# Godotcoffee/AlignGraph2

Hardware: AMD Instinct MI355X
Metric: aligned-read-bases/sec through PAGraph build+traverse (higher is better)
Workload: dtype u32

## Files before the change

aligngraph2_amd/csrc/hip/k2_sort.hip:

```cpp
#include <stdlib.h>

#include "pag_device.hpp"

namespace pagdev {

#ifndef SORT_ST
#define SORT_ST 1024
#endif
#ifndef SORT_ROUNDS
#define SORT_ROUNDS 5
#endif
constexpr int ST = SORT_ST;
constexpr int SW = ST / 64;
constexpr int SROUNDS = SORT_ROUNDS;
constexpr int STILE = ST * SROUNDS;
constexpr int SMAXR = 256;

constexpr int HT = 256;
constexpr int HW = HT / 64;
constexpr int HV = STILE / (4 * HT);
static_assert(STILE % (4 * HT) == 0, "a tile is a whole number of 16-byte loads per thread");

__global__ __launch_bounds__(HT) void sort_hist(const uint32_t *__restrict__ keys, uint64_t n, int shift, uint32_t rmask,
                                                uint32_t *__restrict__ hist, uint32_t n_tiles, int aligned) {
    __shared__ uint32_t h[2][HW][SMAXR];
    const uint32_t w = threadIdx.x >> 6;
    uint4 nx[HV];
    auto request = [&](uint32_t tile) {
        const uint64_t base = (uint64_t)tile * STILE;
        if (aligned && tile < n_tiles && base + STILE <= n) {
            const uint4 *src = (const uint4 *)(keys + base);
#pragma unroll
            for (int r = 0; r < HV; ++r) nx[r] = src[r * HT + threadIdx.x];
        }
    };
    for (uint32_t i = threadIdx.x; i < 2 * HW * SMAXR; i += HT) (&h[0][0][0])[i] = 0;
    request(blockIdx.x);
    __syncthreads();
    uint32_t buf = 0;
    for (uint32_t tile = blockIdx.x; tile < n_tiles; tile += gridDim.x, buf ^= 1u) {
        const uint64_t base = (uint64_t)tile * STILE;
        uint32_t *hw = h[buf][w];
        if (aligned && base + STILE <= n) {
            uint4 cur[HV];
#pragma unroll
            for (int r = 0; r < HV; ++r) cur[r] = nx[r];
            request(tile + gridDim.x);
#pragma unroll
            for (int r = 0; r < HV; ++r) {
                atomicAdd(&hw[(cur[r].x >> shift) & rmask], 1u);
                atomicAdd(&hw[(cur[r].y >> shift) & rmask], 1u);
                atomicAdd(&hw[(cur[r].z >> shift) & rmask], 1u);
                atomicAdd(&hw[(cur[r].w >> shift) & rmask], 1u);
            }
        } else {
            request(tile + gridDim.x);
            for (uint32_t j = threadIdx.x; j < (uint32_t)STILE; j += HT)
                if (base + j < n) atomicAdd(&hw[(keys[base + j] >> shift) & rmask], 1u);
        }
        __syncthreads();
        for (uint32_t d = threadIdx.x; d <= rmask; d += HT) {
            uint32_t c = 0;
#pragma unroll
            for (int ww = 0; ww < HW; ++ww) {
                c += h[buf][ww][d];
                h[buf][ww][d] = 0;
            }
            hist[(uint64_t)d * n_tiles + tile] = c;
        }
    }
}

struct ScatterStage {
    uint64_t goff[SMAXR];
    uint32_t skey[STILE];
#ifdef SORT_TWO_PLANE
    uint32_t sval_lo[STILE], sval_hi[STILE];
#else
    uint64_t sval[STILE];
#endif
};
struct ScatterLds {
    uint32_t wcnt[SW][SMAXR + 1];
    uint32_t dstart[SMAXR];
    ScatterStage stage[2];
};
static_assert(SW == 16 || SW == 8, "the wave prefix below scans groups of SW lanes inside a DPP row");
static_assert(sizeof(ScatterLds) <= 160 * 1024, "LDS");
static_assert(STILE >= SW * SMAXR, "match words alias the payload staging buffer");

__device__ __forceinline__ uint32_t group_incl_sum(uint32_t v, uint32_t pos) {
    uint32_t t;
    t = (uint32_t)__builtin_amdgcn_update_dpp(0, (int)v, 0x111, 0xF, 0xF, true);
    v += (SW == 16 || pos >= 1u) ? t : 0u;
    t = (uint32_t)__builtin_amdgcn_update_dpp(0, (int)v, 0x112, 0xF, 0xF, true);
    v += (SW == 16 || pos >= 2u) ? t : 0u;
    t = (uint32_t)__builtin_amdgcn_update_dpp(0, (int)v, 0x114, 0xF, 0xF, true);
    v += (SW == 16 || pos >= 4u) ? t : 0u;
    if (SW == 16) v += (uint32_t)__builtin_amdgcn_update_dpp(0, (int)v, 0x118, 0xF, 0xF, true);
    return v;
}

__device__ __forceinline__ uint64_t scatter_tile(uint32_t block, uint32_t n_blocks, uint32_t it) {
    if (n_blocks % 8u != 0u) return (uint64_t)it * n_blocks + block;
    const uint32_t per_xcd = n_blocks / 8u, x = block & 7u, slot = block >> 3;
    return ((uint64_t)it * 8u + x) * per_xcd + slot;
}

#ifdef SORT_WAVES_PER_EU
#define SORT_BOUNDS __launch_bounds__(ST, SORT_WAVES_PER_EU)
#else
#define SORT_BOUNDS __launch_bounds__(ST)
#endif
template <int BITS>
__global__ SORT_BOUNDS void sort_scatter(const uint32_t *__restrict__ keys, const uint64_t *__restrict__ vals,
                                                  uint32_t *__restrict__ okeys, uint64_t *__restrict__ ovals, uint64_t n,
                                                  int shift, const uint64_t *__restrict__ hist_scan, uint32_t n_tiles) {
    __shared__ ScatterLds L;
    constexpr uint32_t rmask = (1u << BITS) - 1u;
    const uint32_t lane = lane_id(), w = threadIdx.x >> 6;
    const uint32_t n_iter = (n_tiles + gridDim.x - 1) / gridDim.x;

    uint32_t nkey[SROUNDS];
    uint64_t nval[SROUNDS];
    uint64_t ngbase = 0;
    auto request = [&](uint64_t tile) {
        const uint64_t wb = tile * STILE + (uint64_t)w * (64 * SROUNDS);
        if (threadIdx.x <= rmask && tile < n_tiles) ngbase = hist_scan[(uint64_t)threadIdx.x * n_tiles + tile];
#pragma unroll
        for (int r = 0; r < SROUNDS; ++r) {
            const uint64_t i = wb + (uint64_t)r * 64 + lane;
            const bool valid = tile < n_tiles && i < n;
            nkey[r] = valid ? keys[i] : 0u;
            nval[r] = valid ? vals[i] : 0ull;
        }
    };
    request(scatter_tile(blockIdx.x, gridDim.x, 0));

    const uint32_t last_count = (uint32_t)(n - (uint64_t)(n_tiles - 1u) * STILE);
    auto write_out = [&](const ScatterStage &B, uint32_t count) {
        if (count == (uint32_t)STILE) {
#pragma unroll
            for (int r = 0; r < SROUNDS; ++r) {
                const uint32_t p = (uint32_t)r * ST + threadIdx.x;
                const uint32_t kx = B.skey[p];
                const uint64_t dst = B.goff[(kx >> shift) & rmask] + p;
                okeys[dst] = kx;
#ifdef SORT_TWO_PLANE
                ovals[dst] = (uint64_t)B.sval_lo[p] | ((uint64_t)B.sval_hi[p] << 32);
#else
                ovals[dst] = B.sval[p];
#endif
            }
        } else {
            for (uint32_t p = threadIdx.x; p < count; p += ST) {
                const uint32_t kx = B.skey[p];
                const uint64_t dst = B.goff[(kx >> shift) & rmask] + p;
                okeys[dst] = kx;
#ifdef SORT_TWO_PLANE
                ovals[dst] = (uint64_t)B.sval_lo[p] | ((uint64_t)B.sval_hi[p] << 32);
#else
                ovals[dst] = B.sval[p];
#endif
            }
        }
    };

    bool pending = false;
    uint32_t pending_count = 0;
    uint32_t buf = 0;
    for (uint32_t it = 0; it < n_iter; ++it) {
        const uint64_t tile = scatter_tile(blockIdx.x, gridDim.x, it);
        uint32_t key[SROUNDS];
        uint64_t val[SROUNDS];
#pragma unroll
        for (int r = 0; r < SROUNDS; ++r) {
            key[r] = nkey[r];
            val[r] = nval[r];
        }
        const uint64_t gbase = ngbase;
        if (it + 1 < n_iter) request(scatter_tile(blockIdx.x, gridDim.x, it + 1));
        if (pending) write_out(L.stage[buf ^ 1u], pending_count);
        pending = false;
        if (tile >= n_tiles) continue;

        ScatterStage &B = L.stage[buf];
        const uint64_t tile_base = tile * STILE;
        const uint64_t wave_base = tile_base + (uint64_t)w * (64 * SROUNDS);
#ifdef SORT_TWO_PLANE
        unsigned long long *match = (unsigned long long *)&B.sval_lo[0] + (size_t)w * (rmask + 1u);
#else
        unsigned long long *match = (unsigned long long *)&B.sval[0] + (size_t)w * (rmask + 1u);
#endif
#pragma unroll
        for (int i = 0; i < SMAXR / 64; ++i) L.wcnt[w][i * 64 + lane] = 0;
#pragma unroll
        for (uint32_t i = lane; i <= rmask; i += 64) match[i] = 0ull;
        uint32_t rk[SROUNDS];
#pragma unroll
        for (int r = 0; r < SROUNDS; ++r) {
            const uint64_t i = wave_base + (uint64_t)r * 64 + lane;
            const bool valid = i < n;
            const uint32_t d = (key[r] >> shift) & rmask;
            if (valid) atomicOr(&match[d], 1ull << lane);
            const uint64_t peers = valid ? match[d] : 0ull;
            if (valid) match[d] = 0ull;
            const uint32_t before = __popcll(peers & lanemask_lt());
            const uint32_t base = valid ? L.wcnt[w][d] : 0u;
            if (valid && before == 0) L.wcnt[w][d] = base + (uint32_t)__popcll(peers);
            rk[r] = base + before;
        }

        __syncthreads();
        uint32_t *dtot = (uint32_t *)&B.goff[0];
#pragma unroll
        for (int j = 0; j < SMAXR * SW / ST; ++j) {
            const uint32_t d = (uint32_t)j * (ST / SW) + threadIdx.x / SW, ww = threadIdx.x % SW;
            const uint32_t c = L.wcnt[ww][d];
            const uint32_t incl = group_incl_sum(c, ww);
            L.wcnt[ww][d] = incl - c;
            if (ww == SW - 1u) dtot[d] = incl;
        }
        __syncthreads();
        if (w == 0) {
            const uint32_t t0 = dtot[4 * lane], t1 = dtot[4 * lane + 1], t2 = dtot[4 * lane + 2], t3 = dtot[4 * lane + 3];
            uint32_t tot;
            const uint32_t ex = wave_excl_sum(t0 + t1 + t2 + t3, &tot);
            L.dstart[4 * lane] = ex;
            L.dstart[4 * lane + 1] = ex + t0;
            L.dstart[4 * lane + 2] = ex + t0 + t1;
            L.dstart[4 * lane + 3] = ex + t0 + t1 + t2;
        }
        __syncthreads();
#ifdef SORT_LOOKBACK_PROBE
        if (threadIdx.x <= rmask) {
            uint32_t *rows = (uint32_t *)(hist_scan + (uint64_t)(rmask + 1u) * n_tiles);
            __hip_atomic_store(&rows[tile * (rmask + 1u) + threadIdx.x], dtot[threadIdx.x] | 0x40000000u, __ATOMIC_RELAXED, __HIP_MEMORY_SCOPE_AGENT);
            uint32_t acc = 0;
            for (uint32_t b = 1; b <= (uint32_t)SORT_LOOKBACK_PROBE; ++b) {
                const uint64_t t2 = tile >= b ? tile - b : 0;
                acc += __hip_atomic_load(&rows[t2 * (rmask + 1u) + threadIdx.x], __ATOMIC_RELAXED, __HIP_MEMORY_SCOPE_AGENT);
            }
            if (acc == 0xFFFFFFFFu) L.dstart[threadIdx.x] += 1u;
        }
        __syncthreads();
#endif
        if (threadIdx.x <= rmask) B.goff[threadIdx.x] = gbase - L.dstart[threadIdx.x];

#pragma unroll
        for (int r = 0; r < SROUNDS; ++r) {
            const uint64_t i = wave_base + (uint64_t)r * 64 + lane;
            if (i < n) {
                const uint32_t d = (key[r] >> shift) & rmask;
                const uint32_t p = L.dstart[d] + L.wcnt[w][d] + rk[r];
                B.skey[p] = key[r];
#ifdef SORT_TWO_PLANE
                B.sval_lo[p] = (uint32_t)val[r];
                B.sval_hi[p] = (uint32_t)(val[r] >> 32);
#else
                B.sval[p] = val[r];
#endif
            }
        }
        __syncthreads();
        pending = true;
        pending_count = tile == (uint64_t)n_tiles - 1u ? last_count : (uint32_t)STILE;
        buf ^= 1u;
    }
    if (pending) write_out(L.stage[buf ^ 1u], pending_count);
}

static int scatter_blocks_cus(int dev) {
    static int cus_of[64] = {0};
    int &c = cus_of[dev & 63];
    if (c == 0 && hipDeviceGetAttribute(&c, hipDeviceAttributeMultiprocessorCount, dev) != hipSuccess) c = 256;
    return c > 0 ? c : 256;
}

static size_t sort_align256(size_t x) { return (x + 255) & ~(size_t)255; }

size_t sort_tmp_bytes(uint64_t n) {
    uint64_t n_tiles = (n + STILE - 1) / STILE;
    if (n_tiles == 0) n_tiles = 1;
    uint64_t cells = (uint64_t)SMAXR * n_tiles;
#ifdef SORT_LOOKBACK_PROBE
    return sort_align256(cells * 4) + 2 * sort_align256(cells * 8) + sort_align256(scan_tmp_bytes(cells)) + 256;
#else
    return sort_align256(cells * 4) + sort_align256(cells * 8) + sort_align256(scan_tmp_bytes(cells)) + 256;
#endif
}

int sort_pairs(uint32_t *k0, uint64_t *v0, uint32_t *k1, uint64_t *v1, uint64_t n, int key_bits, void *tmp,
               int *result_in_0, hipStream_t s, float *ms_dominant_kernel, int *n_passes, int first_bit) {
    *result_in_0 = 1;
    if (ms_dominant_kernel) *ms_dominant_kernel = 0.f;
    if (n_passes) *n_passes = 0;
    if (n == 0 || key_bits <= 0) return PAG_OK;
    uint64_t n_tiles64 = (n + STILE - 1) / STILE;
    if (n_tiles64 > 0x7FFFFFFFull) {
        set_error("sort: too many tiles");
        return PAG_EINVAL;
    }
    uint32_t n_tiles = (uint32_t)n_tiles64;
    int passes = (key_bits + 7) / 8;
    int bits = (key_bits + passes - 1) / passes;
    char *p = (char *)tmp;
    uint32_t *hist = (uint32_t *)p;
    uint64_t cells = (uint64_t)SMAXR * n_tiles;
    p += sort_align256(cells * 4);
    uint64_t *hist_scan = (uint64_t *)p;
    p += sort_align256(cells * 8);
    void *scan_tmp = p;

    static int scatter_blocks_of[64] = {0};
    int dev = 0;
    PAG_HIP_TRY(hipGetDevice(&dev));
    int &scatter_blocks = scatter_blocks_of[dev & 63];
    if (scatter_blocks == 0) {
        int cus = 0, per_cu = 0;
        PAG_HIP_TRY(hipDeviceGetAttribute(&cus, hipDeviceAttributeMultiprocessorCount, dev));
        PAG_HIP_TRY(hipOccupancyMaxActiveBlocksPerMultiprocessor(&per_cu, sort_scatter<8>, ST, 0));
        scatter_blocks = cus * (per_cu > 0 ? per_cu : 1);
    }
    const uint32_t scatter_grid = n_tiles < (uint32_t)scatter_blocks ? n_tiles : (uint32_t)scatter_blocks;
    const int hist_per_cu = 8;
    const int hist_blocks = scatter_blocks_cus(dev) * hist_per_cu;
    const bool timed = ms_dominant_kernel != nullptr;
    static thread_local hipEvent_t ev_sets[64][2 * 8];
    static thread_local bool ev_ready[64] = {false};
    hipEvent_t *ev = ev_sets[dev & 63];
    if (timed && !ev_ready[dev & 63]) {
        for (int i = 0; i < 2 * 8; ++i) PAG_HIP_TRY(hipEventCreate(&ev[i]));
        ev_ready[dev & 63] = true;
    }
    uint32_t *ka = k0, *kb = k1;
    uint64_t *va = v0, *vb = v1;
    int in0 = 1;
    for (int pass = 0; pass < passes; ++pass) {
        int shift = first_bit + pass * bits;
        int b = key_bits - pass * bits < bits ? key_bits - pass * bits : bits;
        uint32_t rmask = (1u << b) - 1u;
        uint64_t used = (uint64_t)(rmask + 1) * n_tiles;
        const uint32_t hist_grid = n_tiles < (uint32_t)hist_blocks ? n_tiles : (uint32_t)hist_blocks;
        sort_hist<<<dim3(hist_grid), dim3(HT), 0, s>>>(ka, n, shift, rmask, hist, n_tiles, ((uintptr_t)ka & 15u) == 0 ? 1 : 0);
        int rc = scan_u32_to_u64(hist, hist_scan, used, nullptr, scan_tmp, s);
        if (rc != PAG_OK) return rc;
        if (timed) PAG_HIP_TRY(hipEventRecord(ev[2 * pass], s));
        switch (b) {
#define PAG_SCATTER(B)                                                                                              \
    case B:                                                                                                         \
        sort_scatter<B><<<dim3(scatter_grid), dim3(ST), 0, s>>>(ka, va, kb, vb, n, shift, hist_scan, n_tiles);      \
        break;
            PAG_SCATTER(1) PAG_SCATTER(2) PAG_SCATTER(3) PAG_SCATTER(4) PAG_SCATTER(5) PAG_SCATTER(6) PAG_SCATTER(7) PAG_SCATTER(8)
#undef PAG_SCATTER
        }
        if (timed) PAG_HIP_TRY(hipEventRecord(ev[2 * pass + 1], s));
        uint32_t *tk = ka;
        ka = kb;
        kb = tk;
        uint64_t *tv = va;
        va = vb;
        vb = tv;
        in0 = !in0;
    }
    PAG_HIP_TRY(hipGetLastError());
    if (timed) {
        PAG_HIP_TRY(hipStreamSynchronize(s));
        float tot = 0.f;
        for (int pass = 0; pass < passes; ++pass) {
            float ms = 0.f;
            PAG_HIP_TRY(hipEventElapsedTime(&ms, ev[2 * pass], ev[2 * pass + 1]));
            tot += ms;
        }
        *ms_dominant_kernel = tot / passes;
    }
    if (n_passes) *n_passes = passes;
    *result_in_0 = in0;
    return PAG_OK;
}

}
```

aligngraph2_amd/csrc/hip/k5_travel_host.hip:

```cpp
#include <algorithm>
#include <atomic>
#include <chrono>
#include <cmath>
#include <cstdio>
#include <cstdlib>
#include <cstring>
#include <deque>
#include <string>
#include <thread>
#include <unordered_set>
#include <vector>

#include "pag_graph_impl.hpp"
#include "walk_config.hpp"
#include "walk_stitch.hpp"
#include "walker_grid.hpp"

using namespace pagdev;

namespace {

#include "trav_prepare_host.hpp"
#include "walk_session_jobs.hpp"
#include "walk_session_rounds.hpp"
#include "walk_session_loop.hpp"


}


extern "C" {

uint64_t pag_debug_edit_distance(const char *a, const char *b) { return edit_distance(a, b); }
uint64_t pag_debug_mapper_d2s(const uint32_t *len, uint64_t n, int64_t idx, int64_t pos) { return Mapper(len, n).dualToSingle(idx, pos); }
void pag_debug_mapper_s2d(const uint32_t *len, uint64_t n, uint64_t single, int64_t *idx, int64_t *pos) {
    auto d = Mapper(len, n).singleToDual(single);
    *idx = d.first;
    *pos = d.second;
}
uint64_t pag_debug_mapper_extra(const uint32_t *len, uint64_t n) { return Mapper(len, n).starts.back(); }

const pag_path_node *pag_travel_path_oriented(const pag_graph *g, uint64_t ctg_index, int forward, uint64_t *len) {
    const uint64_t slot = 2 * ctg_index + (forward ? 0 : 1);
    if (!g || slot >= g->path_valid.size() || !g->path_valid[slot]) {
        if (len) *len = 0;
        return nullptr;
    }
    if (len) *len = g->path_len[slot];
    if (slot < g->path_ptr.size() && g->path_ptr[slot]) return g->path_ptr[slot];
    return g->path_store + g->path_off[slot];
}

const char *pag_travel_dump_text(const pag_graph *g, uint64_t ctg_index, int forward, uint64_t *bytes) {
    const uint64_t slot = 2 * ctg_index + (forward ? 0 : 1);
    if (bytes) *bytes = 0;
    if (!g || slot >= g->path_valid.size() || !g->path_valid[slot] || slot >= g->text_ptr.size() || !g->text_ptr[slot]) return nullptr;
    if (bytes) *bytes = g->text_len[slot];
    return g->text_ptr[slot];
}

const pag_path_node *pag_travel_path(const pag_graph *g, uint64_t ctg_index, uint64_t *len) {
    if (g && 2 * ctg_index + 1 < g->path_valid.size() && !g->path_valid[2 * ctg_index]) return pag_travel_path_oriented(g, ctg_index, 0, len);
    return pag_travel_path_oriented(g, ctg_index, 1, len);
}

int pag_debug_succ_sizes(const pag_graph *g, uint64_t *n_pos, uint64_t *n_succ) {
    if (!g || !g->tg_ready || !n_pos || !n_succ) return PAG_EINVAL;
    *n_pos = g->tg.n_pos;
    *n_succ = g->tg.n_succ;
    return PAG_OK;
}
int pag_debug_succ(const pag_graph *g, uint32_t *succ_off, void *recs) {
    if (!g || !g->tg_ready || !succ_off || !recs) return PAG_EINVAL;
    PAG_HIP_TRY(hipSetDevice(g->device));
    PAG_HIP_TRY(hipMemcpy(succ_off, g->tg.succ_off, (g->tg.n_pos + 1) * 4, hipMemcpyDeviceToHost));
    PAG_HIP_TRY(hipMemcpy(recs, g->tg.succ, g->tg.n_succ * sizeof(SuccRec), hipMemcpyDeviceToHost));
    return PAG_OK;
}

int pag_debug_trav_vertices(const pag_graph *g, uint32_t *code, uint64_t *pos) {
    if (!g || !g->tg_ready || !code || !pos) return PAG_EINVAL;
    PAG_HIP_TRY(hipSetDevice(g->device));
    const TravGraph &G = g->tg;
    std::vector<uint32_t> uold(G.n_pos), vnode(G.n_pos), ncode(G.n_nodes);
    PAG_HIP_TRY(hipMemcpy(uold.data(), G.uold, G.n_pos * 4, hipMemcpyDeviceToHost));
    PAG_HIP_TRY(hipMemcpy(vnode.data(), G.vnode, G.n_pos * 4, hipMemcpyDeviceToHost));
    PAG_HIP_TRY(hipMemcpy(ncode.data(), G.ncode, G.n_nodes * 4, hipMemcpyDeviceToHost));
    PAG_HIP_TRY(hipMemcpy(pos, G.upos, G.n_pos * 8, hipMemcpyDeviceToHost));
    for (uint64_t u = 0; u < G.n_pos; ++u) code[u] = ncode[vnode[uold[u]]];
    return PAG_OK;
}

int64_t pag_successors(const pag_graph *g, uint32_t code, uint64_t pos, pag_succ *out, uint64_t cap) {
    if (!g || !g->tg_ready || (!out && cap)) return PAG_EINVAL;
    PAG_HIP_TRY(hipSetDevice(g->device));
    if (g->view_pruned || g->regional) {
        set_error("pag_successors: the prepared view was cut for given traversals (pag_travel_prepare_for / a regional graph): its lists are restricted to what those traversals can examine");
        return PAG_ERANGE;
    }
    void *d = nullptr;
    const uint64_t room = std::min<uint64_t>(cap, g->tg.n_succ);
    PAG_HIP_TRY(hipMalloc(&d, 16 + room * sizeof(pag_succ)));
    unsigned long long *d_n = (unsigned long long *)d;
    void *d_recs = (char *)d + 16;
    int rc = trav_successors_of(g->tg, code, pos, d_recs, room, d_n, g->stream);
    unsigned long long n = 0;
    if (rc == PAG_OK && (hipMemcpyAsync(&n, d_n, 8, hipMemcpyDeviceToHost, g->stream) != hipSuccess || hipStreamSynchronize(g->stream) != hipSuccess)) rc = PAG_EFAULT;
    if (rc == PAG_OK && n == ~0ull) {
        set_error("pag_successors: the graph holds no vertex with that k-mer and position");
        rc = PAG_EINVAL;
    } else if (rc == PAG_OK && n == ~1ull) {
        set_error("pag_successors: that vertex's list is a marker record");
        rc = PAG_ERANGE;
    } else if (rc == PAG_OK && std::min<uint64_t>(n, room) &&
               hipMemcpy(out, d_recs, std::min<uint64_t>(n, room) * sizeof(pag_succ), hipMemcpyDeviceToHost) != hipSuccess) {
        rc = PAG_EFAULT;
    }
    hipFree(d);
    return rc == PAG_OK ? (int64_t)n : rc;
}

int pag_travel_prepare(pag_graph *g, const pag_seqs *ctgs, const uint32_t *ref_len, uint64_t n_refs, const pag_travel_params *prm, double *ms) {
    return pag_travel_prepare_for(g, ctgs, nullptr, ref_len, n_refs, prm, ms);
}
int pag_travel_prepare_for(pag_graph *g, const pag_seqs *ctgs, const int32_t *orient, const uint32_t *ref_len, uint64_t n_refs,
                           const pag_travel_params *prm, double *ms) {
    if (!g || !ctgs || !prm || (!ref_len && n_refs)) return PAG_EINVAL;
    PAG_HIP_TRY(hipSetDevice(g->device));
    TravGraph G{};
    return trav_prepare_graph(g, ctgs->len, ctgs->n_seqs, ref_len, n_refs, prm->deviation, prm->error_rate, &G, ms, orient, prm->start_split);
}
int pag_travel_view_sizes(const pag_graph *g, uint64_t *n_nodes, uint64_t *n_pos, uint64_t *n_edges, uint64_t *n_succ, int *cut, uint64_t *fallbacks) {
    if (!g || !g->tg_ready) return PAG_EINVAL;
    if (n_nodes) *n_nodes = g->view_counts[0];
    if (n_pos) *n_pos = g->view_counts[1];
    if (n_edges) *n_edges = g->view_counts[2];
    if (n_succ) *n_succ = g->tg.n_succ;
    if (cut) *cut = g->view_pruned ? 1 : 0;
    if (fallbacks) *fallbacks = g->view_fallbacks;
    return PAG_OK;
}

static int travel_once(pag_graph *g, const pag_seqs *ctgs, const int32_t *orient, const uint32_t *ref_len, uint64_t n_refs,
                       const pag_travel_params *prm, pag_travel_stats *stats);
int pag_travel(pag_graph *g, const pag_seqs *ctgs, const int32_t *orient, const uint32_t *ref_len, uint64_t n_refs,
               const pag_travel_params *prm, pag_travel_stats *stats) {
    if (!g || !ctgs || !orient || !prm || (!ref_len && n_refs)) return PAG_EINVAL;
    int rc = travel_once(g, ctgs, orient, ref_len, n_refs, prm, stats);
    if (rc == PAG_ERANGE && g->view_pruned && !g->regional) {
        if (WalkConfig::from_env().timing) std::fprintf(stderr, "[timing] a walk left the view: %s; walking again on the whole graph\n", pag_last_error());
        g->view_off = true;
        g->tg_ready = false;
        g->view_fallbacks += 1;
        rc = travel_once(g, ctgs, orient, ref_len, n_refs, prm, stats);
    }
    return rc;
}
static int travel_once(pag_graph *g, const pag_seqs *ctgs, const int32_t *orient, const uint32_t *ref_len, uint64_t n_refs,
                       const pag_travel_params *prm, pag_travel_stats *stats) {
    WalkSession W(g, ctgs, orient, ref_len, n_refs, prm, stats);
    return W.run();
}


}
```

aligngraph2_amd/csrc/hip/k5_view.hip:

```cpp
#include <algorithm>
#include <cmath>
#include <cstring>
#include <string>
#include <vector>

#include "pag_device.hpp"
#include "pag_travel.hpp"
#include "trav_device.hpp"

namespace pagdev {

__device__ __forceinline__ bool iv_contains(const uint32_t *__restrict__ iv, uint32_t n, uint32_t x, uint32_t *which = nullptr) {
    if (!n) return false;
    uint32_t lo = 0, hi = n;
    while (hi - lo > 1) {
        const uint32_t mid = (lo + hi) >> 1;
        if (iv[2 * mid] <= x) lo = mid;
        else hi = mid;
    }
    if (which) *which = lo;
    return x >= iv[2 * lo] && x < iv[2 * lo + 1];
}
constexpr uint32_t ZONE_LDS = 2048;
__global__ void k_zone_bands(const uint64_t *__restrict__ tval, uint64_t T, const uint32_t *__restrict__ zones, uint32_t n_z,
                             uint32_t *__restrict__ lo, uint32_t *__restrict__ hi) {
    __shared__ uint32_t s_lo[ZONE_LDS], s_hi[ZONE_LDS], s_z[2 * ZONE_LDS];
    const bool lds = n_z <= ZONE_LDS;
    if (lds) {
        for (uint32_t z = threadIdx.x; z < n_z; z += blockDim.x) {
            s_lo[z] = 0xFFFFFFFFu;
            s_hi[z] = 0u;
            s_z[2 * z] = zones[2 * z];
            s_z[2 * z + 1] = zones[2 * z + 1];
        }
        __syncthreads();
    }
    const uint32_t z_first = n_z ? zones[0] : 0u, z_last = n_z ? zones[2 * n_z - 1] : 0u;
    for (uint64_t i = (uint64_t)blockIdx.x * blockDim.x + threadIdx.x; i < T; i += (uint64_t)gridDim.x * blockDim.x) {
        const uint64_t p = tval[i];
        const uint32_t c = (uint32_t)(p >> 32), r = (uint32_t)p;
        uint32_t z;
        if (c < z_first || c >= z_last || r == 0u) continue;
        if (!(lds ? iv_contains(s_z, n_z, c, &z) : iv_contains(zones, n_z, c, &z))) continue;
        if (lds) {
            atomicMin(&s_lo[z], r);
            atomicMax(&s_hi[z], r);
        } else {
            atomicMin(&lo[z], r);
            atomicMax(&hi[z], r);
        }
    }
    if (lds) {
        __syncthreads();
        for (uint32_t z = threadIdx.x; z < n_z; z += blockDim.x)
            if (s_hi[z] != 0u) {
                atomicMin(&lo[z], s_lo[z]);
                atomicMax(&hi[z], s_hi[z]);
            }
    }
}
constexpr uint32_t PRUNE_LDS = 4096;
constexpr uint32_t VC_T = 256, VC_R = 8, VC_TILE = VC_T * VC_R, VC_W = VC_T / 64;
__global__ __launch_bounds__(VC_T) void k_view_mark(const uint32_t *__restrict__ tkey, const uint64_t *__restrict__ tval, const uint32_t *__restrict__ tseg,
                                                    uint64_t T, const uint32_t *__restrict__ civ, uint32_t n_civ, const uint32_t *__restrict__ riv,
                                                    uint32_t n_riv, int whole, uint64_t *__restrict__ ballots, uint32_t *__restrict__ tile_first,
                                                    uint32_t *__restrict__ tile_keep, uint64_t n_tiles) {
    __shared__ uint32_t s_iv[PRUNE_LDS];
    __shared__ uint32_t s_ck[VC_R][VC_W], s_pk[VC_R][VC_W], s_cf[VC_R][VC_W];
    __shared__ uint16_t s_pre[VC_TILE];
    const bool lds = !whole && 2u * (n_civ + n_riv) <= PRUNE_LDS;
    if (lds) {
        for (uint32_t x = threadIdx.x; x < 2u * n_civ; x += blockDim.x) s_iv[x] = civ[x];
        for (uint32_t x = threadIdx.x; x < 2u * n_riv; x += blockDim.x) s_iv[2u * n_civ + x] = riv[x];
        __syncthreads();
    }
    auto inside = [&](uint64_t p) {
        const uint32_t c = (uint32_t)(p >> 32), r = (uint32_t)p;
        if (whole) return true;
        if (lds) return c != 0u ? iv_contains(s_iv, n_civ, c) : iv_contains(s_iv + 2u * n_civ, n_riv, r);
        return c != 0u ? iv_contains(civ, n_civ, c) : iv_contains(riv, n_riv, r);
    };
    const uint32_t lane = lane_id(), w = threadIdx.x >> 6;
    for (uint64_t tile = blockIdx.x; tile < n_tiles; tile += gridDim.x) {
        const uint64_t tile_base = tile * VC_TILE;
        uint32_t kb = 0;
        uint32_t off_r[VC_R];
        uint64_t bkr[VC_R];
#pragma unroll
        for (uint32_t r = 0; r < VC_R; ++r) {
            const uint64_t i = tile_base + (uint64_t)r * VC_T + threadIdx.x;
            bool kk = false;
            off_r[r] = 0;
            if (i < T) {
                const uint32_t kx = tkey[i], v = tseg[i];
                const bool head = i == 0 || tkey[i - 1] != kx;
                const bool leader = head ? v != 0u : (v & SEG_LEADER) != 0u;
                if (leader) {
                    kk = inside(tval[i]);
                    off_r[r] = head ? 0u : (v & ~SEG_LEADER);
                }
            }
            bkr[r] = __ballot(kk);
            kb |= kk ? 1u << r : 0u;
            if (lane == 0) s_ck[r][w] = (uint32_t)__popcll(bkr[r]);
        }
        __syncthreads();
        if (threadIdx.x == 0) {
            uint32_t ak = 0;
            for (uint32_t r = 0; r < VC_R; ++r)
                for (uint32_t ww = 0; ww < VC_W; ++ww) {
                    s_pk[r][ww] = ak;
                    ak += s_ck[r][ww];
                }
            tile_keep[tile] = ak;
        }
        __syncthreads();
#pragma unroll
        for (uint32_t r = 0; r < VC_R; ++r)
            s_pre[r * VC_T + threadIdx.x] = (uint16_t)(s_pk[r][w] + (uint32_t)__popcll(bkr[r] & lanemask_lt()));
        __syncthreads();
#pragma unroll
        for (uint32_t r = 0; r < VC_R; ++r) {
            const uint32_t d = r * VC_T + threadIdx.x;
            bool ff = false;
            if ((kb >> r) & 1u) {
                const uint32_t off = off_r[r];
                if (off <= d) {
                    ff = s_pre[d] == s_pre[d - off];
                } else {
                    ff = s_pre[d] == 0u;
                    const uint64_t i = tile_base + d;
                    for (uint64_t j = i - off; j < tile_base && ff; ++j) {
                        const uint32_t kx = tkey[j], v = tseg[j];
                        const bool head = j == 0 || tkey[j - 1] != kx;
                        const bool leader = head ? v != 0u : (v & SEG_LEADER) != 0u;
                        ff = !(leader && inside(tval[j]));
                    }
                }
            }
            const uint64_t bf = __ballot(ff);
            if (lane == 0) {
                s_cf[r][w] = (uint32_t)__popcll(bf);
                const uint64_t at = ((tile * VC_R + r) * VC_W + w) * 2u;
                ballots[at] = bkr[r];
                ballots[at + 1] = bf;
            }
        }
        __syncthreads();
        if (threadIdx.x == 0) {
            uint32_t af = 0;
            for (uint32_t r = 0; r < VC_R; ++r)
                for (uint32_t ww = 0; ww < VC_W; ++ww) af += s_cf[r][ww];
            tile_first[tile] = af;
        }
    }
}
__global__ __launch_bounds__(VC_T) void k_view_write(const uint32_t *__restrict__ tkey, const uint64_t *__restrict__ tval, const uint16_t *__restrict__ tcnt,
                                                     const uint64_t *__restrict__ ballots, const uint64_t *__restrict__ base_first,
                                                     const uint64_t *__restrict__ base_keep, uint64_t n_tiles, TravGraph G) {
    __shared__ uint64_t s_b[VC_R * VC_W * 2];
    __shared__ uint32_t s_pk[VC_R][VC_W], s_pf[VC_R][VC_W];
    const uint32_t w = threadIdx.x >> 6;
    for (uint64_t tile = blockIdx.x; tile < n_tiles; tile += gridDim.x) {
        if (threadIdx.x < VC_R * VC_W * 2) s_b[threadIdx.x] = ballots[tile * (VC_R * VC_W * 2) + threadIdx.x];
        __syncthreads();
        if (threadIdx.x == 0) {
            uint32_t ak = 0, af = 0;
            for (uint32_t r = 0; r < VC_R; ++r)
                for (uint32_t ww = 0; ww < VC_W; ++ww) {
                    s_pk[r][ww] = ak;
                    s_pf[r][ww] = af;
                    ak += (uint32_t)__popcll(s_b[(r * VC_W + ww) * 2]);
                    af += (uint32_t)__popcll(s_b[(r * VC_W + ww) * 2 + 1]);
                }
        }
        __syncthreads();
        const uint64_t bk0 = base_keep[tile], bf0 = base_first[tile];
#pragma unroll
        for (uint32_t r = 0; r < VC_R; ++r) {
            const uint64_t bk = s_b[(r * VC_W + w) * 2], bf = s_b[(r * VC_W + w) * 2 + 1];
            const uint64_t me = 1ull << lane_id();
            if (!(bk & me)) continue;
            const bool ff = (bf & me) != 0ull;
            const uint64_t i = tile * VC_TILE + (uint64_t)r * VC_T + threadIdx.x;
            const uint64_t p = bk0 + s_pk[r][w] + (uint32_t)__popcll(bk & lanemask_lt());
            const uint64_t n = bf0 + s_pf[r][w] + (uint32_t)__popcll(bf & lanemask_lt()) + (ff ? 1u : 0u) - 1u;
            G.vpos[p] = tval[i];
            G.vcnt[p] = tcnt[i];
            G.vnode[p] = (uint32_t)n;
            if (ff) {
                const uint32_t kx = tkey[i];
                G.ncode[n] = kx;
                G.npos_off[n] = (uint32_t)p;
                atomicOr((unsigned long long *)&G.bitmap[kx >> 6], 1ull << (kx & 63u));
            }
        }
        __syncthreads();
    }
}

__global__ void k_popc_words(const uint64_t *__restrict__ bitmap, uint64_t n_words, uint32_t *__restrict__ out) {
    for (uint64_t i = (uint64_t)blockIdx.x * blockDim.x + threadIdx.x; i < n_words; i += (uint64_t)gridDim.x * blockDim.x)
        out[i] = (uint32_t)__popcll(bitmap[i]);
}

__global__ void k_narrow(const uint64_t *__restrict__ in, uint64_t n, uint32_t *__restrict__ out) {
    for (uint64_t i = (uint64_t)blockIdx.x * blockDim.x + threadIdx.x; i < n; i += (uint64_t)gridDim.x * blockDim.x)
        out[i] = (uint32_t)in[i];
}

__global__ void k_edge_counts(const uint32_t *__restrict__ ekey, const uint32_t *__restrict__ eseg, uint64_t E, TravGraph G,
                              uint32_t *__restrict__ necnt) {
    for (uint64_t j = (uint64_t)blockIdx.x * blockDim.x + threadIdx.x; j < E; j += (uint64_t)gridDim.x * blockDim.x) {
        uint32_t kx = ekey[j];
        if (j != 0 && ekey[j - 1] == kx) continue;
        uint32_t n = node_of_code(G, kx);
        if (n != PAG_NONE) necnt[n] = eseg[j];
    }
}

__global__ void k_code_table(TravGraph G, uint64_t *__restrict__ tab) {
    for (uint64_t n = (uint64_t)blockIdx.x * blockDim.x + threadIdx.x; n < G.n_nodes; n += (uint64_t)gridDim.x * blockDim.x) {
        const U32x2 r = *(const U32x2 *)(G.npos_off + n);
        tab[G.ncode[n]] = (uint64_t)r.a[0] | ((uint64_t)(r.a[1] - r.a[0]) << 32);
    }
}

__global__ void k_compact_edges(const uint32_t *__restrict__ ekey, const uint64_t *__restrict__ eval,
                                const uint32_t *__restrict__ eseg, uint64_t E, TravGraph G, const uint64_t *__restrict__ tab) {
    for (uint64_t j = (uint64_t)blockIdx.x * blockDim.x + threadIdx.x; j < E; j += (uint64_t)gridDim.x * blockDim.x) {
        uint32_t kx = ekey[j];
        if (j != 0 && ekey[j - 1] == kx) continue;
        uint32_t n = node_of_code(G, kx);
        if (n == PAG_NONE) continue;
        uint32_t dst = G.nedge_off[n], len = eseg[j];
        for (uint32_t l0 = 0; l0 < len; l0 += 4u) {
            uint64_t v4[4];
            uint32_t p04[4], q4[4];
#pragma unroll
            for (uint32_t t = 0; t < 4u; ++t) v4[t] = l0 + t < len ? eval[j + l0 + t] : 0ull;
            if (tab) {
                uint64_t e4[4];
#pragma unroll
                for (uint32_t t = 0; t < 4u; ++t) e4[t] = l0 + t < len ? tab[(uint32_t)(v4[t] >> 32)] : ~0ull;
#pragma unroll
                for (uint32_t t = 0; t < 4u; ++t) {
                    p04[t] = (uint32_t)e4[t];
                    q4[t] = (uint32_t)(e4[t] >> 32);
                }
            } else {
                uint32_t to4[4];
                U32x2 r4[4];
#pragma unroll
                for (uint32_t t = 0; t < 4u; ++t) to4[t] = l0 + t < len ? node_of_code(G, (uint32_t)(v4[t] >> 32)) : PAG_NONE;
#pragma unroll
                for (uint32_t t = 0; t < 4u; ++t) r4[t] = *(const U32x2 *)(G.npos_off + (to4[t] != PAG_NONE ? to4[t] : 0u));
#pragma unroll
                for (uint32_t t = 0; t < 4u; ++t) {
                    p04[t] = to4[t] != PAG_NONE ? r4[t].a[0] : PAG_NONE;
                    q4[t] = r4[t].a[1] - r4[t].a[0];
                }
            }
#pragma unroll
            for (uint32_t t = 0; t < 4u; ++t) {
                const uint32_t l = l0 + t;
                if (l >= len) break;
                const uint32_t step = (((uint32_t)v4[t]) >> 1) & EDGE_STEP_MASK;
                if (p04[t] == PAG_NONE) {
                    G.eto[dst + l] = PAG_NONE;
                    G.estep[dst + l] = step;
                } else {
                    G.eto[dst + l] = p04[t];
                    G.estep[dst + l] = step | ((q4[t] < EDGE_Q_MANY ? q4[t] : EDGE_Q_MANY) << 24);
                }
            }
        }
    }
}

__global__ void k_ctg_nodes(const uint8_t *__restrict__ packed, const TravCtgNodesJob *__restrict__ jobs, uint32_t k, TravGraph G,
                            uint32_t *__restrict__ out_all) {
    const TravCtgNodesJob J = jobs[blockIdx.y];
    const uint32_t len = J.len;
    const bool forward = J.forward != 0;
    uint32_t *__restrict__ out = out_all + J.out_off;
    const uint32_t n_pos = len >= k ? len - k + 1 : 0;
    const uint32_t kmask = k >= 16 ? 0xFFFFFFFFu : ((1u << (2 * k)) - 1u);
    const uint32_t *words = (const uint32_t *)(packed + J.byte_off);
    for (uint32_t i = blockIdx.x * blockDim.x + threadIdx.x; i < n_pos; i += gridDim.x * blockDim.x) {
        uint32_t a = forward ? i : len - k - i;
        uint32_t w = a >> 4, sh = (a & 15u) * 2u;
        uint64_t W = (uint64_t)words[w] | ((uint64_t)words[w + 1] << 32);
        uint32_t x = (uint32_t)(W >> sh) & kmask;
        uint32_t code = forward ? (rev2(x) >> (32 - 2 * k)) : ((~x) & kmask);
        out[i] = node_of_code(G, code);
    }
}

__global__ void k_order_keys(const uint64_t *__restrict__ vpos, uint64_t n, uint32_t *__restrict__ key, uint64_t *__restrict__ val) {
    for (uint64_t i = (uint64_t)blockIdx.x * blockDim.x + threadIdx.x; i < n; i += (uint64_t)gridDim.x * blockDim.x) {
        const uint64_t p = vpos[i];
        key[i] = (uint32_t)(p >> 32);
        val[i] = (p << 32) | i;
    }
}

__global__ void k_order_apply(const uint32_t *__restrict__ sorted_ctg, const uint64_t *__restrict__ sorted_val, uint64_t n, uint64_t n_zero, TravGraph G,
                              uint32_t slice, uint32_t slice_shift) {
    for (uint64_t u = (uint64_t)blockIdx.x * blockDim.x + threadIdx.x; u < n; u += (uint64_t)gridDim.x * blockDim.x) {
        uint32_t v;
        if (slice == 0u) {
            const uint64_t x = sorted_val[u];
            v = (uint32_t)x;
            G.uold[u] = v;
            G.upos[u] = ((uint64_t)(u < n_zero ? 0u : sorted_ctg[u]) << 32) | (x >> 32);
        } else {
            v = G.uold[u];
        }
        if (slice_shift >= 32u || (v >> slice_shift) == slice) {
            G.newid[v] = (uint32_t)u;
            G.ucnt[u] = G.vcnt[v];
        }
    }
}

int trav_compact(const uint32_t *tkey, const uint64_t *tval, const uint32_t *tseg, const uint16_t *tcnt, uint64_t T,
                 const uint32_t *ekey, const uint64_t *eval, const uint32_t *eseg, uint64_t E, uint32_t k, uint64_t n_nodes,
                 uint64_t n_pos, uint64_t n_edges, TravGraph G, void *tmp, size_t tmp_bytes, hipStream_t s, const TravView *view,
                 uint64_t *counts_out) {
    const uint64_t n_words = ((1ull << (2 * k)) + 63) / 64;
    const uint64_t n_tiles_all = (T + VC_TILE - 1) / VC_TILE;
    const uint64_t m = std::max(n_tiles_all, std::max(n_words, n_nodes + 1)) + 1;
    const uint64_t m_ballots = n_tiles_all * (VC_TILE / 64 * 2 + 1) + 64;
    char *p = (char *)tmp;
    auto take = [&](size_t bytes) {
        char *q = p;
        p += (bytes + 255) & ~(size_t)255;
        return (void *)q;
    };
    uint32_t *flags = (uint32_t *)take(m * 4);
    uint64_t *sc1 = (uint64_t *)take(m * 8);
    uint64_t *sc2 = (uint64_t *)take(m_ballots * 8);
    uint32_t *keep = (uint32_t *)take((n_tiles_all + 1) * 4);
    uint64_t *totals = (uint64_t *)take(64);
    void *scan_tmp = take(scan_tmp_bytes(m));
    uint64_t *code_tab = k <= TRAV_CODE_TABLE_MAX_K ? (uint64_t *)take((size_t)8 << (2 * k)) : nullptr;
    if ((size_t)(p - (char *)tmp) > tmp_bytes) {
        set_error("trav_compact: scratch too small");
        return PAG_EINVAL;
    }
    PAG_HIP_TRY(hipMemsetAsync(G.bitmap, 0, n_words * 8, s));
    int rc;
    if (T) {
        const uint64_t n_tiles = (T + VC_TILE - 1) / VC_TILE;
        uint32_t *tile_first = flags, *tile_keep = keep;
        const unsigned grid = (unsigned)std::min<uint64_t>(n_tiles, 256u * 8u);
        const uint32_t *civ = view ? view->civ : nullptr, *riv = view ? view->riv : nullptr;
        const uint32_t n_civ = view ? view->n_civ : 0u, n_riv = view ? view->n_riv : 0u;
        uint64_t *ballots = sc2 + n_tiles + 16;
        k_view_mark<<<dim3(grid), dim3(VC_T), 0, s>>>(tkey, tval, tseg, T, civ, n_civ, riv, n_riv, view ? 0 : 1, ballots, tile_first, tile_keep, n_tiles);
        if ((rc = scan_u32_to_u64(tile_first, sc1, n_tiles, totals, scan_tmp, s))) return rc;
        if ((rc = scan_u32_to_u64(tile_keep, sc2, n_tiles, totals + 1, scan_tmp, s))) return rc;
        k_view_write<<<dim3(grid), dim3(VC_T), 0, s>>>(tkey, tval, tcnt, ballots, sc1, sc2, n_tiles, G);
    }
    if (view) {
        uint64_t h[2] = {0, 0};
        if (T) {
            PAG_HIP_TRY(hipMemcpyAsync(h, totals, 16, hipMemcpyDeviceToHost, s));
            PAG_HIP_TRY(hipStreamSynchronize(s));
        }
        if (h[0] > n_nodes || h[1] > n_pos) {
            set_error("trav_compact: the view holds more than the graph");
            return PAG_EFAULT;
        }
        n_nodes = h[0];
        n_pos = h[1];
        G.n_nodes = n_nodes;
        G.n_pos = n_pos;
    }
    uint32_t np32 = (uint32_t)n_pos;
    PAG_HIP_TRY(hipMemcpyAsync(G.npos_off + n_nodes, &np32, 4, hipMemcpyHostToDevice, s));
    k_popc_words<<<dim3(grid_for(n_words)), dim3(256), 0, s>>>(G.bitmap, n_words, flags);
    if ((rc = scan_u32_to_u64(flags, sc1, n_words, nullptr, scan_tmp, s))) return rc;
    k_narrow<<<dim3(grid_for(n_words)), dim3(256), 0, s>>>(sc1, n_words, G.rank);
    PAG_HIP_TRY(hipMemsetAsync(flags, 0, (n_nodes + 1) * 4, s));
    if (E) k_edge_counts<<<dim3(grid_for(E)), dim3(256), 0, s>>>(ekey, eseg, E, G, flags);
    if ((rc = scan_u32_to_u64(flags, sc1, n_nodes + 1, view ? totals + 2 : nullptr, scan_tmp, s))) return rc;
    k_narrow<<<dim3(grid_for(n_nodes + 1)), dim3(256), 0, s>>>(sc1, n_nodes + 1, G.nedge_off);
    if (E && code_tab) {
        PAG_HIP_TRY(hipMemsetAsync(code_tab, 0xFF, (size_t)8 << (2 * k), s));
        TravGraph Gn = G;
        Gn.n_nodes = n_nodes;
        if (n_nodes) k_code_table<<<dim3(grid_for(n_nodes)), dim3(256), 0, s>>>(Gn, code_tab);
    }
    if (E) k_compact_edges<<<dim3(grid_for(E)), dim3(256), 0, s>>>(ekey, eval, eseg, E, G, code_tab);
    if (view) {
        uint64_t ne = 0;
        PAG_HIP_TRY(hipMemcpyAsync(&ne, totals + 2, 8, hipMemcpyDeviceToHost, s));
        PAG_HIP_TRY(hipStreamSynchronize(s));
        if (ne > n_edges) {
            set_error("trav_compact: the view holds more edges than the graph");
            return PAG_EFAULT;
        }
        n_edges = ne;
    }
    if (counts_out) {
        counts_out[0] = n_nodes;
        counts_out[1] = n_pos;
        counts_out[2] = n_edges;
    }
    PAG_HIP_TRY(hipGetLastError());
    return PAG_OK;
}

size_t trav_compact_tmp_bytes(uint64_t T, uint64_t E, uint32_t k, uint64_t n_nodes) {
    (void)E;
    const uint64_t n_words = ((1ull << (2 * k)) + 63) / 64;
    const uint64_t n_tiles = (T + VC_TILE - 1) / VC_TILE;
    const uint64_t m = std::max(n_tiles, std::max(n_words, n_nodes + 1)) + 1, m_ballots = n_tiles * (VC_TILE / 64 * 2 + 1) + 64;
    auto al = [](size_t b) { return (b + 255) & ~(size_t)255; };
    return al(m * 4) + al(m * 8) + al(m_ballots * 8) + al((n_tiles + 1) * 4) + al(64) + al(scan_tmp_bytes(m)) + (k <= TRAV_CODE_TABLE_MAX_K ? al((size_t)8 << (2 * k)) : 0) + 1024;
}

int trav_zone_bands(const uint64_t *tval, uint64_t T, const uint32_t *zones_dev, uint32_t n_z, uint32_t *lo_dev, uint32_t *hi_dev, hipStream_t s) {
    if (!n_z) return PAG_OK;
    PAG_HIP_TRY(hipMemsetAsync(lo_dev, 0xFF, (size_t)n_z * 4, s));
    PAG_HIP_TRY(hipMemsetAsync(hi_dev, 0, (size_t)n_z * 4, s));
    if (T) k_zone_bands<<<dim3(grid_for(T)), dim3(256), 0, s>>>(tval, T, zones_dev, n_z, lo_dev, hi_dev);
    PAG_HIP_TRY(hipGetLastError());
    return PAG_OK;
}

void trav_launch_ctg_nodes(const uint8_t *packed, const TravCtgNodesJob *jobs, uint32_t n_jobs, uint32_t max_len, uint32_t k, TravGraph G, uint32_t *out,
                           hipStream_t s) {
    const uint32_t n = max_len >= k ? max_len - k + 1 : 0;
    if (!n || !n_jobs) return;
    for (uint32_t at = 0; at < n_jobs; at += 65535u) {
        const uint32_t m = std::min(n_jobs - at, 65535u);
        k_ctg_nodes<<<dim3(std::min(grid_for(n), 256u), m), dim3(256), 0, s>>>(packed, jobs + at, k, G, out);
    }
}

__global__ void k_max_step(const uint32_t *__restrict__ estep, uint64_t n, uint32_t *__restrict__ out) {
    uint32_t m = 0;
    for (uint64_t i = (uint64_t)blockIdx.x * blockDim.x + threadIdx.x; i < n; i += (uint64_t)gridDim.x * blockDim.x) m = (estep[i] & EDGE_STEP_MASK) > m ? (estep[i] & EDGE_STEP_MASK) : m;
    m = wave_max_u32(m);
    if (lane_id() == 0 && m) atomicMax(out, m);
}
__global__ void k_mark_incomplete(TravGraph G, uint32_t n_zero, const uint32_t *__restrict__ iv, const uint8_t *__restrict__ open, uint32_t n_iv,
                                  uint32_t margin, uint32_t *__restrict__ bits) {
    const uint64_t u = (uint64_t)blockIdx.x * blockDim.x + threadIdx.x;
    bool bad = false;
    if (u < G.n_pos) bad = d_incomplete_by_position(iv, open, n_iv, margin, (uint32_t)G.upos[u], u >= n_zero);
    const uint64_t m = __ballot(bad);
    if ((threadIdx.x & 63u) == 0 && u < ((G.n_pos + 63ull) & ~63ull)) {
        bits[u >> 5] = (uint32_t)m;
        bits[(u >> 5) + 1] = (uint32_t)(m >> 32);
    }
}
int trav_mark_incomplete(TravGraph &G, uint32_t n_zero, const uint32_t *iv_host, const uint8_t *open_host, uint32_t n_iv, uint32_t dev, double err,
                         uint32_t *bits, void *tmp, hipStream_t s) {
    uint32_t *d_max = (uint32_t *)tmp;
    uint32_t *d_iv = d_max + 64;
    uint8_t *d_open = (uint8_t *)(d_iv + 2 * (size_t)n_iv + 2);
    PAG_HIP_TRY(hipMemsetAsync(d_max, 0, 4, s));
    if (G.n_edges) k_max_step<<<dim3(grid_for(G.n_edges)), dim3(256), 0, s>>>(G.estep, G.n_edges, d_max);
    if (n_iv) {
        PAG_HIP_TRY(hipMemcpyAsync(d_iv, iv_host, 2 * (size_t)n_iv * 4, hipMemcpyHostToDevice, s));
        PAG_HIP_TRY(hipMemcpyAsync(d_open, open_host, 2 * (size_t)n_iv, hipMemcpyHostToDevice, s));
    }
    uint32_t max_step = 0;
    PAG_HIP_TRY(hipMemcpyAsync(&max_step, d_max, 4, hipMemcpyDeviceToHost, s));
    PAG_HIP_TRY(hipStreamSynchronize(s));
    const uint64_t margin = (uint64_t)((double)max_step * (1.0 + err)) + dev + 2;
    const bool bits_read = n_iv > INC_LDS_MAX;
    if (G.n_pos && bits_read) k_mark_incomplete<<<dim3((unsigned)((G.n_pos + 255) / 256)), dim3(256), 0, s>>>(G, n_zero, d_iv, d_open, n_iv, (uint32_t)std::min<uint64_t>(margin, 0x7FFFFFFFu), bits);
    PAG_HIP_TRY(hipGetLastError());
    G.incomplete = bits;
    G.inc_iv = d_iv;
    G.inc_open = d_open;
    G.inc_n = n_iv;
    G.inc_margin = (uint32_t)std::min<uint64_t>(margin, 0x7FFFFFFFu);
    return PAG_OK;
}
size_t trav_mark_incomplete_tmp_bytes(uint32_t n_iv) { return 256 + (2 * (size_t)n_iv + 2) * 4 + 2 * (size_t)n_iv + 64; }

__global__ void k_zero_prefix(const uint32_t *__restrict__ key, uint64_t n, unsigned long long *__restrict__ n0) {
    for (uint64_t i = (uint64_t)blockIdx.x * blockDim.x + threadIdx.x; i < n; i += (uint64_t)gridDim.x * blockDim.x)
        if (key[i] == 0u && (i + 1 == n || key[i + 1] != 0u)) *n0 = i + 1;
}
__global__ void k_order_refkeys(const uint64_t *__restrict__ val, uint64_t n, uint32_t *__restrict__ key) {
    for (uint64_t i = (uint64_t)blockIdx.x * blockDim.x + threadIdx.x; i < n; i += (uint64_t)gridDim.x * blockDim.x)
        key[i] = (uint32_t)(val[i] >> 32);
}

int trav_order(TravGraph G, uint32_t *key, uint64_t *val, uint32_t *key2, uint64_t *val2, void *sort_tmp, uint64_t *n_zero, int ctg_bits,
               int ref_bits, hipStream_t s) {
    const uint64_t n = G.n_pos;
    if (n_zero) *n_zero = 0;
    if (!n) return PAG_OK;
    k_order_keys<<<dim3(grid_for(n)), dim3(256), 0, s>>>(G.vpos, n, key, val);
    int in0 = 1, rc;
    if ((rc = sort_pairs(key, val, key2, val2, n, ctg_bits, sort_tmp, &in0, s, nullptr, nullptr))) return rc;
    uint32_t *ks = in0 ? key : key2, *ko = in0 ? key2 : key;
    uint64_t *vs = in0 ? val : val2, *vo = in0 ? val2 : val;
    unsigned long long *d_n0 = (unsigned long long *)sort_tmp;
    unsigned long long n0 = 0;
    PAG_HIP_TRY(hipMemsetAsync(d_n0, 0, 8, s));
    k_zero_prefix<<<dim3(grid_for(n)), dim3(256), 0, s>>>(ks, n, d_n0);
    PAG_HIP_TRY(hipMemcpyAsync(&n0, d_n0, 8, hipMemcpyDeviceToHost, s));
    PAG_HIP_TRY(hipStreamSynchronize(s));
    if (n0 > 1) {
        k_order_refkeys<<<dim3(grid_for(n0)), dim3(256), 0, s>>>(vs, n0, ks);
        int in0b = 1;
        if ((rc = sort_pairs(ks, vs, ko, vo, n0, ref_bits, sort_tmp, &in0b, s, nullptr, nullptr))) return rc;
        if (!in0b) PAG_HIP_TRY(hipMemcpyAsync(vs, vo, n0 * 8, hipMemcpyDeviceToDevice, s));
    }
    if (n_zero) *n_zero = n0;
    {
        uint32_t lg = n >= (32ull << 20) ? 3u : 0u;
        if (const long long want = env_int("PAG_ORDER_SLICES", 0)) {
            lg = 0;
            while ((1u << (lg + 1)) <= (uint32_t)std::max<long long>(1, want)) ++lg;
        }
        uint32_t bits = 1;
        while (bits < 32 && (n >> bits) != 0) ++bits;
        if (lg >= bits) lg = 0;
        const uint32_t shift = lg ? bits - lg : 32u;
        for (uint32_t sl = 0; sl < (1u << lg); ++sl)
            k_order_apply<<<dim3(grid_for(n)), dim3(256), 0, s>>>(ks, vs, n, n0 > 1 ? n0 : 0, G, sl, shift);
    }
    PAG_HIP_TRY(hipGetLastError());
    return PAG_OK;
}

}
```

Before: 4.188 billion.

## Template radix sort on input/output adapters to fuse key packing into first and last passes

Moves the radix sort kernels into a header and templates the histogram and scatter kernels on input and output adapter types. A sort can then read keys directly from a source layout on its first pass and write a final layout on its last pass, instead of running separate pack and unpack kernels. This appears aimed at the coordinate-ordering path, removing extra full-array passes around the sort. It adds template complexity and a debug entry point, and plain sort_pairs keeps the array adapters.

New measurement: 3.972 billion. -5.2%, worse.

```diff
diff --git a/aligngraph2_amd/csrc/hip/k2_sort.hip b/aligngraph2_amd/csrc/hip/k2_sort.hip
--- a/aligngraph2_amd/csrc/hip/k2_sort.hip
+++ b/aligngraph2_amd/csrc/hip/k2_sort.hip
@@ -1,274 +1,9 @@
 #include <stdlib.h>
 
 #include "pag_device.hpp"
+#include "sort_kernels.hpp"
 
 namespace pagdev {
-
-#ifndef SORT_ST
-#define SORT_ST 1024
-#endif
-#ifndef SORT_ROUNDS
-#define SORT_ROUNDS 5
-#endif
-constexpr int ST = SORT_ST;
-constexpr int SW = ST / 64;
-constexpr int SROUNDS = SORT_ROUNDS;
-constexpr int STILE = ST * SROUNDS;
-constexpr int SMAXR = 256;
-
-constexpr int HT = 256;
-constexpr int HW = HT / 64;
-constexpr int HV = STILE / (4 * HT);
-static_assert(STILE % (4 * HT) == 0, "a tile is a whole number of 16-byte loads per thread");
-
-__global__ __launch_bounds__(HT) void sort_hist(const uint32_t *__restrict__ keys, uint64_t n, int shift, uint32_t rmask,
-                                                uint32_t *__restrict__ hist, uint32_t n_tiles, int aligned) {
-    __shared__ uint32_t h[2][HW][SMAXR];
-    const uint32_t w = threadIdx.x >> 6;
-    uint4 nx[HV];
-    auto request = [&](uint32_t tile) {
-        const uint64_t base = (uint64_t)tile * STILE;
-        if (aligned && tile < n_tiles && base + STILE <= n) {
-            const uint4 *src = (const uint4 *)(keys + base);
-#pragma unroll
-            for (int r = 0; r < HV; ++r) nx[r] = src[r * HT + threadIdx.x];
-        }
-    };
-    for (uint32_t i = threadIdx.x; i < 2 * HW * SMAXR; i += HT) (&h[0][0][0])[i] = 0;
-    request(blockIdx.x);
-    __syncthreads();
-    uint32_t buf = 0;
-    for (uint32_t tile = blockIdx.x; tile < n_tiles; tile += gridDim.x, buf ^= 1u) {
-        const uint64_t base = (uint64_t)tile * STILE;
-        uint32_t *hw = h[buf][w];
-        if (aligned && base + STILE <= n) {
-            uint4 cur[HV];
-#pragma unroll
-            for (int r = 0; r < HV; ++r) cur[r] = nx[r];
-            request(tile + gridDim.x);
-#pragma unroll
-            for (int r = 0; r < HV; ++r) {
-                atomicAdd(&hw[(cur[r].x >> shift) & rmask], 1u);
-                atomicAdd(&hw[(cur[r].y >> shift) & rmask], 1u);
-                atomicAdd(&hw[(cur[r].z >> shift) & rmask], 1u);
-                atomicAdd(&hw[(cur[r].w >> shift) & rmask], 1u);
-            }
-        } else {
-            request(tile + gridDim.x);
-            for (uint32_t j = threadIdx.x; j < (uint32_t)STILE; j += HT)
-                if (base + j < n) atomicAdd(&hw[(keys[base + j] >> shift) & rmask], 1u);
-        }
-        __syncthreads();
-        for (uint32_t d = threadIdx.x; d <= rmask; d += HT) {
-            uint32_t c = 0;
-#pragma unroll
-            for (int ww = 0; ww < HW; ++ww) {
-                c += h[buf][ww][d];
-                h[buf][ww][d] = 0;
-            }
-            hist[(uint64_t)d * n_tiles + tile] = c;
-        }
-    }
-}
-
-struct ScatterStage {
-    uint64_t goff[SMAXR];
-    uint32_t skey[STILE];
-#ifdef SORT_TWO_PLANE
-    uint32_t sval_lo[STILE], sval_hi[STILE];
-#else
-    uint64_t sval[STILE];
-#endif
-};
-struct ScatterLds {
-    uint32_t wcnt[SW][SMAXR + 1];
-    uint32_t dstart[SMAXR];
-    ScatterStage stage[2];
-};
-static_assert(SW == 16 || SW == 8, "the wave prefix below scans groups of SW lanes inside a DPP row");
-static_assert(sizeof(ScatterLds) <= 160 * 1024, "LDS");
-static_assert(STILE >= SW * SMAXR, "match words alias the payload staging buffer");
-
-__device__ __forceinline__ uint32_t group_incl_sum(uint32_t v, uint32_t pos) {
-    uint32_t t;
-    t = (uint32_t)__builtin_amdgcn_update_dpp(0, (int)v, 0x111, 0xF, 0xF, true);
-    v += (SW == 16 || pos >= 1u) ? t : 0u;
-    t = (uint32_t)__builtin_amdgcn_update_dpp(0, (int)v, 0x112, 0xF, 0xF, true);
-    v += (SW == 16 || pos >= 2u) ? t : 0u;
-    t = (uint32_t)__builtin_amdgcn_update_dpp(0, (int)v, 0x114, 0xF, 0xF, true);
-    v += (SW == 16 || pos >= 4u) ? t : 0u;
-    if (SW == 16) v += (uint32_t)__builtin_amdgcn_update_dpp(0, (int)v, 0x118, 0xF, 0xF, true);
-    return v;
-}
-
-__device__ __forceinline__ uint64_t scatter_tile(uint32_t block, uint32_t n_blocks, uint32_t it) {
-    if (n_blocks % 8u != 0u) return (uint64_t)it * n_blocks + block;
-    const uint32_t per_xcd = n_blocks / 8u, x = block & 7u, slot = block >> 3;
-    return ((uint64_t)it * 8u + x) * per_xcd + slot;
-}
-
-#ifdef SORT_WAVES_PER_EU
-#define SORT_BOUNDS __launch_bounds__(ST, SORT_WAVES_PER_EU)
-#else
-#define SORT_BOUNDS __launch_bounds__(ST)
-#endif
-template <int BITS>
-__global__ SORT_BOUNDS void sort_scatter(const uint32_t *__restrict__ keys, const uint64_t *__restrict__ vals,
-                                                  uint32_t *__restrict__ okeys, uint64_t *__restrict__ ovals, uint64_t n,
-                                                  int shift, const uint64_t *__restrict__ hist_scan, uint32_t n_tiles) {
-    __shared__ ScatterLds L;
-    constexpr uint32_t rmask = (1u << BITS) - 1u;
-    const uint32_t lane = lane_id(), w = threadIdx.x >> 6;
-    const uint32_t n_iter = (n_tiles + gridDim.x - 1) / gridDim.x;
-
-    uint32_t nkey[SROUNDS];
-    uint64_t nval[SROUNDS];
-    uint64_t ngbase = 0;
-    auto request = [&](uint64_t tile) {
-        const uint64_t wb = tile * STILE + (uint64_t)w * (64 * SROUNDS);
-        if (threadIdx.x <= rmask && tile < n_tiles) ngbase = hist_scan[(uint64_t)threadIdx.x * n_tiles + tile];
-#pragma unroll
-        for (int r = 0; r < SROUNDS; ++r) {
-            const uint64_t i = wb + (uint64_t)r * 64 + lane;
-            const bool valid = tile < n_tiles && i < n;
-            nkey[r] = valid ? keys[i] : 0u;
-            nval[r] = valid ? vals[i] : 0ull;
-        }
-    };
-    request(scatter_tile(blockIdx.x, gridDim.x, 0));
-
-    const uint32_t last_count = (uint32_t)(n - (uint64_t)(n_tiles - 1u) * STILE);
-    auto write_out = [&](const ScatterStage &B, uint32_t count) {
-        if (count == (uint32_t)STILE) {
-#pragma unroll
-            for (int r = 0; r < SROUNDS; ++r) {
-                const uint32_t p = (uint32_t)r * ST + threadIdx.x;
-                const uint32_t kx = B.skey[p];
-                const uint64_t dst = B.goff[(kx >> shift) & rmask] + p;
-                okeys[dst] = kx;
-#ifdef SORT_TWO_PLANE
-                ovals[dst] = (uint64_t)B.sval_lo[p] | ((uint64_t)B.sval_hi[p] << 32);
-#else
-                ovals[dst] = B.sval[p];
-#endif
-            }
-        } else {
-            for (uint32_t p = threadIdx.x; p < count; p += ST) {
-                const uint32_t kx = B.skey[p];
-                const uint64_t dst = B.goff[(kx >> shift) & rmask] + p;
-                okeys[dst] = kx;
-#ifdef SORT_TWO_PLANE
-                ovals[dst] = (uint64_t)B.sval_lo[p] | ((uint64_t)B.sval_hi[p] << 32);
-#else
-                ovals[dst] = B.sval[p];
-#endif
-            }
-        }
-    };
-
-    bool pending = false;
-    uint32_t pending_count = 0;
-    uint32_t buf = 0;
-    for (uint32_t it = 0; it < n_iter; ++it) {
-        const uint64_t tile = scatter_tile(blockIdx.x, gridDim.x, it);
-        uint32_t key[SROUNDS];
-        uint64_t val[SROUNDS];
-#pragma unroll
-        for (int r = 0; r < SROUNDS; ++r) {
-            key[r] = nkey[r];
-            val[r] = nval[r];
-        }
-        const uint64_t gbase = ngbase;
-        if (it + 1 < n_iter) request(scatter_tile(blockIdx.x, gridDim.x, it + 1));
-        if (pending) write_out(L.stage[buf ^ 1u], pending_count);
-        pending = false;
-        if (tile >= n_tiles) continue;
-
-        ScatterStage &B = L.stage[buf];
-        const uint64_t tile_base = tile * STILE;
-        const uint64_t wave_base = tile_base + (uint64_t)w * (64 * SROUNDS);
-#ifdef SORT_TWO_PLANE
-        unsigned long long *match = (unsigned long long *)&B.sval_lo[0] + (size_t)w * (rmask + 1u);
-#else
-        unsigned long long *match = (unsigned long long *)&B.sval[0] + (size_t)w * (rmask + 1u);
-#endif
-#pragma unroll
-        for (int i = 0; i < SMAXR / 64; ++i) L.wcnt[w][i * 64 + lane] = 0;
-#pragma unroll
-        for (uint32_t i = lane; i <= rmask; i += 64) match[i] = 0ull;
-        uint32_t rk[SROUNDS];
-#pragma unroll
-        for (int r = 0; r < SROUNDS; ++r) {
-            const uint64_t i = wave_base + (uint64_t)r * 64 + lane;
-            const bool valid = i < n;
-            const uint32_t d = (key[r] >> shift) & rmask;
-            if (valid) atomicOr(&match[d], 1ull << lane);
-            const uint64_t peers = valid ? match[d] : 0ull;
-            if (valid) match[d] = 0ull;
-            const uint32_t before = __popcll(peers & lanemask_lt());
-            const uint32_t base = valid ? L.wcnt[w][d] : 0u;
-            if (valid && before == 0) L.wcnt[w][d] = base + (uint32_t)__popcll(peers);
-            rk[r] = base + before;
-        }
-
-        __syncthreads();
-        uint32_t *dtot = (uint32_t *)&B.goff[0];
-#pragma unroll
-        for (int j = 0; j < SMAXR * SW / ST; ++j) {
-            const uint32_t d = (uint32_t)j * (ST / SW) + threadIdx.x / SW, ww = threadIdx.x % SW;
-            const uint32_t c = L.wcnt[ww][d];
-            const uint32_t incl = group_incl_sum(c, ww);
-            L.wcnt[ww][d] = incl - c;
-            if (ww == SW - 1u) dtot[d] = incl;
-        }
-        __syncthreads();
-        if (w == 0) {
-            const uint32_t t0 = dtot[4 * lane], t1 = dtot[4 * lane + 1], t2 = dtot[4 * lane + 2], t3 = dtot[4 * lane + 3];
-            uint32_t tot;
-            const uint32_t ex = wave_excl_sum(t0 + t1 + t2 + t3, &tot);
-            L.dstart[4 * lane] = ex;
-            L.dstart[4 * lane + 1] = ex + t0;
-            L.dstart[4 * lane + 2] = ex + t0 + t1;
-            L.dstart[4 * lane + 3] = ex + t0 + t1 + t2;
-        }
-        __syncthreads();
-#ifdef SORT_LOOKBACK_PROBE
-        if (threadIdx.x <= rmask) {
-            uint32_t *rows = (uint32_t *)(hist_scan + (uint64_t)(rmask + 1u) * n_tiles);
-            __hip_atomic_store(&rows[tile * (rmask + 1u) + threadIdx.x], dtot[threadIdx.x] | 0x40000000u, __ATOMIC_RELAXED, __HIP_MEMORY_SCOPE_AGENT);
-            uint32_t acc = 0;
-            for (uint32_t b = 1; b <= (uint32_t)SORT_LOOKBACK_PROBE; ++b) {
-                const uint64_t t2 = tile >= b ? tile - b : 0;
-                acc += __hip_atomic_load(&rows[t2 * (rmask + 1u) + threadIdx.x], __ATOMIC_RELAXED, __HIP_MEMORY_SCOPE_AGENT);
-            }
-            if (acc == 0xFFFFFFFFu) L.dstart[threadIdx.x] += 1u;
-        }
-        __syncthreads();
-#endif
-        if (threadIdx.x <= rmask) B.goff[threadIdx.x] = gbase - L.dstart[threadIdx.x];
-
-#pragma unroll
-        for (int r = 0; r < SROUNDS; ++r) {
-            const uint64_t i = wave_base + (uint64_t)r * 64 + lane;
-            if (i < n) {
-                const uint32_t d = (key[r] >> shift) & rmask;
-                const uint32_t p = L.dstart[d] + L.wcnt[w][d] + rk[r];
-                B.skey[p] = key[r];
-#ifdef SORT_TWO_PLANE
-                B.sval_lo[p] = (uint32_t)val[r];
-                B.sval_hi[p] = (uint32_t)(val[r] >> 32);
-#else
-                B.sval[p] = val[r];
-#endif
-            }
-        }
-        __syncthreads();
-        pending = true;
-        pending_count = tile == (uint64_t)n_tiles - 1u ? last_count : (uint32_t)STILE;
-        buf ^= 1u;
-    }
-    if (pending) write_out(L.stage[buf ^ 1u], pending_count);
-}
 
 static int scatter_blocks_cus(int dev) {
     static int cus_of[64] = {0};
@@ -290,28 +25,7 @@
 #endif
 }
 
-int sort_pairs(uint32_t *k0, uint64_t *v0, uint32_t *k1, uint64_t *v1, uint64_t n, int key_bits, void *tmp,
-               int *result_in_0, hipStream_t s, float *ms_dominant_kernel, int *n_passes, int first_bit) {
-    *result_in_0 = 1;
-    if (ms_dominant_kernel) *ms_dominant_kernel = 0.f;
-    if (n_passes) *n_passes = 0;
-    if (n == 0 || key_bits <= 0) return PAG_OK;
-    uint64_t n_tiles64 = (n + STILE - 1) / STILE;
-    if (n_tiles64 > 0x7FFFFFFFull) {
-        set_error("sort: too many tiles");
-        return PAG_EINVAL;
-    }
-    uint32_t n_tiles = (uint32_t)n_tiles64;
-    int passes = (key_bits + 7) / 8;
-    int bits = (key_bits + passes - 1) / passes;
-    char *p = (char *)tmp;
-    uint32_t *hist = (uint32_t *)p;
-    uint64_t cells = (uint64_t)SMAXR * n_tiles;
-    p += sort_align256(cells * 4);
-    uint64_t *hist_scan = (uint64_t *)p;
-    p += sort_align256(cells * 8);
-    void *scan_tmp = p;
-
+int sort_grids(uint32_t *scatter_blocks_out, uint32_t *hist_blocks_out) {
     static int scatter_blocks_of[64] = {0};
     int dev = 0;
     PAG_HIP_TRY(hipGetDevice(&dev));
@@ -322,61 +36,30 @@
         PAG_HIP_TRY(hipOccupancyMaxActiveBlocksPerMultiprocessor(&per_cu, sort_scatter<8>, ST, 0));
         scatter_blocks = cus * (per_cu > 0 ? per_cu : 1);
     }
-    const uint32_t scatter_grid = n_tiles < (uint32_t)scatter_blocks ? n_tiles : (uint32_t)scatter_blocks;
     const int hist_per_cu = 8;
-    const int hist_blocks = scatter_blocks_cus(dev) * hist_per_cu;
-    const bool timed = ms_dominant_kernel != nullptr;
+    *scatter_blocks_out = (uint32_t)scatter_blocks;
+    *hist_blocks_out = (uint32_t)(scatter_blocks_cus(dev) * hist_per_cu);
+    return PAG_OK;
+}
+
+int sort_timing_events(hipEvent_t **ev_out) {
     static thread_local hipEvent_t ev_sets[64][2 * 8];
     static thread_local bool ev_ready[64] = {false};
+    int dev = 0;
+    PAG_HIP_TRY(hipGetDevice(&dev));
     hipEvent_t *ev = ev_sets[dev & 63];
-    if (timed && !ev_ready[dev & 63]) {
+    if (!ev_ready[dev & 63]) {
         for (int i = 0; i < 2 * 8; ++i) PAG_HIP_TRY(hipEventCreate(&ev[i]));
         ev_ready[dev & 63] = true;
     }
-    uint32_t *ka = k0, *kb = k1;
-    uint64_t *va = v0, *vb = v1;
-    int in0 = 1;
-    for (int pass = 0; pass < passes; ++pass) {
-        int shift = first_bit + pass * bits;
-        int b = key_bits - pass * bits < bits ? key_bits - pass * bits : bits;
-        uint32_t rmask = (1u << b) - 1u;
-        uint64_t used = (uint64_t)(rmask + 1) * n_tiles;
-        const uint32_t hist_grid = n_tiles < (uint32_t)hist_blocks ? n_tiles : (uint32_t)hist_blocks;
-        sort_hist<<<dim3(hist_grid), dim3(HT), 0, s>>>(ka, n, shift, rmask, hist, n_tiles, ((uintptr_t)ka & 15u) == 0 ? 1 : 0);
-        int rc = scan_u32_to_u64(hist, hist_scan, used, nullptr, scan_tmp, s);
-        if (rc != PAG_OK) return rc;
-        if (timed) PAG_HIP_TRY(hipEventRecord(ev[2 * pass], s));
-        switch (b) {
-#define PAG_SCATTER(B)                                                                                              \
-    case B:                                                                                                         \
-        sort_scatter<B><<<dim3(scatter_grid), dim3(ST), 0, s>>>(ka, va, kb, vb, n, shift, hist_scan, n_tiles);      \
-        break;
-            PAG_SCATTER(1) PAG_SCATTER(2) PAG_SCATTER(3) PAG_SCATTER(4) PAG_SCATTER(5) PAG_SCATTER(6) PAG_SCATTER(7) PAG_SCATTER(8)
-#undef PAG_SCATTER
-        }
-        if (timed) PAG_HIP_TRY(hipEventRecord(ev[2 * pass + 1], s));
-        uint32_t *tk = ka;
-        ka = kb;
-        kb = tk;
-        uint64_t *tv = va;
-        va = vb;
-        vb = tv;
-        in0 = !in0;
-    }
-    PAG_HIP_TRY(hipGetLastError());
-    if (timed) {
-        PAG_HIP_TRY(hipStreamSynchronize(s));
-        float tot = 0.f;
-        for (int pass = 0; pass < passes; ++pass) {
-            float ms = 0.f;
-            PAG_HIP_TRY(hipEventElapsedTime(&ms, ev[2 * pass], ev[2 * pass + 1]));
-            tot += ms;
-        }
-        *ms_dominant_kernel = tot / passes;
-    }
-    if (n_passes) *n_passes = passes;
-    *result_in_0 = in0;
+    *ev_out = ev;
     return PAG_OK;
 }
 
+int sort_pairs(uint32_t *k0, uint64_t *v0, uint32_t *k1, uint64_t *v1, uint64_t n, int key_bits, void *tmp,
+               int *result_in_0, hipStream_t s, float *ms_dominant_kernel, int *n_passes, int first_bit) {
+    return sort_passes<SortArrayIn, SortArrayOut>(k0, v0, nullptr, nullptr, 0u, k0, v0, k1, v1, n, key_bits, tmp, result_in_0, s, ms_dominant_kernel,
+                                                  n_passes, first_bit, nullptr);
 }
+
+}
diff --git a/aligngraph2_amd/csrc/hip/k5_travel_host.hip b/aligngraph2_amd/csrc/hip/k5_travel_host.hip
--- a/aligngraph2_amd/csrc/hip/k5_travel_host.hip
+++ b/aligngraph2_amd/csrc/hip/k5_travel_host.hip
@@ -88,6 +88,54 @@
     PAG_HIP_TRY(hipMemcpy(ncode.data(), G.ncode, G.n_nodes * 4, hipMemcpyDeviceToHost));
     PAG_HIP_TRY(hipMemcpy(pos, G.upos, G.n_pos * 8, hipMemcpyDeviceToHost));
     for (uint64_t u = 0; u < G.n_pos; ++u) code[u] = ncode[vnode[uold[u]]];
+    return PAG_OK;
+}
+
+int pag_debug_coord_order(const uint64_t *vpos, const uint16_t *vcnt, uint64_t n, int ctg_bits, int ref_bits, int device, int vpos_skew, uint32_t *uold,
+                          uint64_t *upos, uint32_t *newid, uint32_t *ucnt, uint64_t *n_zero) {
+    if (!vpos || !vcnt || !uold || !upos || !newid || !ucnt || !n_zero || n == 0 || n > 0xFFFFFFFFull || ctg_bits < 1 || ctg_bits > 32 || ref_bits < 1 ||
+        ref_bits > 32 || vpos_skew < 0 || vpos_skew > 3)
+        return PAG_EINVAL;
+    PAG_HIP_TRY(hipSetDevice(device));
+    struct Bufs {
+        std::vector<void *> all;
+        ~Bufs() {
+            for (void *p : all) (void)hipFree(p);
+        }
+        void *get(size_t bytes) {
+            void *p = nullptr;
+            if (hipMalloc(&p, bytes + 64) != hipSuccess) return nullptr;
+            all.push_back(p);
+            return p;
+        }
+    } bufs;
+    TravGraph G{};
+    G.n_pos = n;
+    uint64_t *d_vpos = (uint64_t *)bufs.get((n + 4) * 8);
+    G.vcnt = (uint16_t *)bufs.get(n * 2);
+    G.uold = (uint32_t *)bufs.get(n * 4);
+    G.newid = (uint32_t *)bufs.get(n * 4);
+    G.upos = (uint64_t *)bufs.get(n * 8);
+    G.ucnt = (uint32_t *)bufs.get(n * 4);
+    uint32_t *k0 = (uint32_t *)bufs.get((n + 8) * 4), *k1 = (uint32_t *)bufs.get((n + 8) * 4);
+    uint64_t *v0 = (uint64_t *)bufs.get((n + 8) * 8), *v1 = (uint64_t *)bufs.get((n + 8) * 8);
+    void *tmp = bufs.get(sort_tmp_bytes(n));
+    if (!d_vpos || !G.vcnt || !G.uold || !G.newid || !G.upos || !G.ucnt || !k0 || !k1 || !v0 || !v1 || !tmp) {
+        set_error("pag_debug_coord_order: out of device memory");
+        return PAG_ENOMEM;
+    }
+    G.vpos = d_vpos + vpos_skew;
+    PAG_HIP_TRY(hipMemcpy(G.vpos, vpos, n * 8, hipMemcpyHostToDevice));
+    PAG_HIP_TRY(hipMemcpy(G.vcnt, vcnt, n * 2, hipMemcpyHostToDevice));
+    PAG_HIP_TRY(hipMemset(G.newid, 0xFF, n * 4));
+    PAG_HIP_TRY(hipMemset(G.ucnt, 0xFF, n * 4));
+    const int rc = trav_order(G, k0, v0, k1, v1, tmp, n_zero, ctg_bits, ref_bits, nullptr);
+    if (rc != PAG_OK) return rc;
+    PAG_HIP_TRY(hipDeviceSynchronize());
+    PAG_HIP_TRY(hipMemcpy(uold, G.uold, n * 4, hipMemcpyDeviceToHost));
+    PAG_HIP_TRY(hipMemcpy(upos, G.upos, n * 8, hipMemcpyDeviceToHost));
+    PAG_HIP_TRY(hipMemcpy(newid, G.newid, n * 4, hipMemcpyDeviceToHost));
+    PAG_HIP_TRY(hipMemcpy(ucnt, G.ucnt, n * 4, hipMemcpyDeviceToHost));
     return PAG_OK;
 }
 
diff --git a/aligngraph2_amd/csrc/hip/k5_view.hip b/aligngraph2_amd/csrc/hip/k5_view.hip
--- a/aligngraph2_amd/csrc/hip/k5_view.hip
+++ b/aligngraph2_amd/csrc/hip/k5_view.hip
@@ -6,6 +6,7 @@
 
 #include "pag_device.hpp"
 #include "pag_travel.hpp"
+#include "sort_kernels.hpp"
 #include "trav_device.hpp"
 
 namespace pagdev {
@@ -297,6 +298,42 @@
     }
 }
 
+__device__ __forceinline__ uint32_t order_key(uint64_t p, uint32_t B) {
+    const uint32_t ctg = (uint32_t)(p >> 32);
+    return ctg ? (1u << B) | ctg : (uint32_t)p;
+}
+struct OrderIn {
+    typedef uint64_t A;
+    typedef void B;
+    struct Quad {
+        ulonglong2 lo, hi;
+    };
+    static __device__ __forceinline__ Quad quad(const A *a, uint64_t base, uint32_t j) {
+        const ulonglong2 *p = (const ulonglong2 *)(a + base) + 2 * j;
+        return Quad{p[0], p[1]};
+    }
+    static __device__ __forceinline__ void quad_keys(const Quad &x, uint32_t bits, uint32_t (&k)[4]) {
+        k[0] = order_key(x.lo.x, bits);
+        k[1] = order_key(x.lo.y, bits);
+        k[2] = order_key(x.hi.x, bits);
+        k[3] = order_key(x.hi.y, bits);
+    }
+    static __device__ __forceinline__ uint32_t key(const A *a, uint64_t i, uint32_t bits) { return order_key(a[i], bits); }
+    static __device__ __forceinline__ void rec(const A *a, const B *, uint64_t i, uint32_t bits, uint32_t &k, uint64_t &v) {
+        const uint64_t p = a[i];
+        k = order_key(p, bits);
+        v = (p << 32) | i;
+    }
+};
+struct OrderOut {
+    typedef uint32_t A;
+    typedef uint64_t B;
+    static __device__ __forceinline__ void put(A *uold, B *upos, uint64_t dst, uint32_t k, uint64_t v, uint32_t bits) {
+        uold[dst] = (uint32_t)v;
+        upos[dst] = ((uint64_t)((k >> bits) & 1u ? k & ((1u << bits) - 1u) : 0u) << 32) | (v >> 32);
+    }
+};
+
 __global__ void k_order_keys(const uint64_t *__restrict__ vpos, uint64_t n, uint32_t *__restrict__ key, uint64_t *__restrict__ val) {
     for (uint64_t i = (uint64_t)blockIdx.x * blockDim.x + threadIdx.x; i < n; i += (uint64_t)gridDim.x * blockDim.x) {
         const uint64_t p = vpos[i];
@@ -304,19 +341,17 @@
         val[i] = (p << 32) | i;
     }
 }
-
-__global__ void k_order_apply(const uint32_t *__restrict__ sorted_ctg, const uint64_t *__restrict__ sorted_val, uint64_t n, uint64_t n_zero, TravGraph G,
-                              uint32_t slice, uint32_t slice_shift) {
+__global__ void k_order_unpack(const uint32_t *__restrict__ sorted_ctg, const uint64_t *__restrict__ sorted_val, uint64_t n, uint64_t n_zero, TravGraph G) {
     for (uint64_t u = (uint64_t)blockIdx.x * blockDim.x + threadIdx.x; u < n; u += (uint64_t)gridDim.x * blockDim.x) {
-        uint32_t v;
-        if (slice == 0u) {
-            const uint64_t x = sorted_val[u];
-            v = (uint32_t)x;
-            G.uold[u] = v;
-            G.upos[u] = ((uint64_t)(u < n_zero ? 0u : sorted_ctg[u]) << 32) | (x >> 32);
-        } else {
-            v = G.uold[u];
-        }
+        const uint64_t x = sorted_val[u];
+        G.uold[u] = (uint32_t)x;
+        G.upos[u] = ((uint64_t)(u < n_zero ? 0u : sorted_ctg[u]) << 32) | (x >> 32);
+    }
+}
+
+__global__ void k_order_apply(uint64_t n, TravGraph G, uint32_t slice, uint32_t slice_shift) {
+    for (uint64_t u = (uint64_t)blockIdx.x * blockDim.x + threadIdx.x; u < n; u += (uint64_t)gridDim.x * blockDim.x) {
+        const uint32_t v = G.uold[u];
         if (slice_shift >= 32u || (v >> slice_shift) == slice) {
             G.newid[v] = (uint32_t)u;
             G.ucnt[u] = G.vcnt[v];
@@ -499,24 +534,33 @@
     const uint64_t n = G.n_pos;
     if (n_zero) *n_zero = 0;
     if (!n) return PAG_OK;
-    k_order_keys<<<dim3(grid_for(n)), dim3(256), 0, s>>>(G.vpos, n, key, val);
+    const int B = std::max(ctg_bits, ref_bits);
+    const bool merged = B + 1 <= 32 && (B + 1 + 7) / 8 <= (ctg_bits + 7) / 8 && env_int("PAG_ORDER_TWO_SORTS", 0) == 0;
     int in0 = 1, rc;
-    if ((rc = sort_pairs(key, val, key2, val2, n, ctg_bits, sort_tmp, &in0, s, nullptr, nullptr))) return rc;
-    uint32_t *ks = in0 ? key : key2, *ko = in0 ? key2 : key;
-    uint64_t *vs = in0 ? val : val2, *vo = in0 ? val2 : val;
-    unsigned long long *d_n0 = (unsigned long long *)sort_tmp;
     unsigned long long n0 = 0;
-    PAG_HIP_TRY(hipMemsetAsync(d_n0, 0, 8, s));
-    k_zero_prefix<<<dim3(grid_for(n)), dim3(256), 0, s>>>(ks, n, d_n0);
-    PAG_HIP_TRY(hipMemcpyAsync(&n0, d_n0, 8, hipMemcpyDeviceToHost, s));
-    PAG_HIP_TRY(hipStreamSynchronize(s));
-    if (n0 > 1) {
-        k_order_refkeys<<<dim3(grid_for(n0)), dim3(256), 0, s>>>(vs, n0, ks);
-        int in0b = 1;
-        if ((rc = sort_pairs(ks, vs, ko, vo, n0, ref_bits, sort_tmp, &in0b, s, nullptr, nullptr))) return rc;
-        if (!in0b) PAG_HIP_TRY(hipMemcpyAsync(vs, vo, n0 * 8, hipMemcpyDeviceToDevice, s));
-    }
-    if (n_zero) *n_zero = n0;
+    const uint64_t *d_n0 = nullptr;
+    if (merged) {
+        if ((rc = sort_passes<OrderIn, OrderOut>(G.vpos, nullptr, G.uold, G.upos, (uint32_t)B, key, val, key2, val2, n, B + 1, sort_tmp, &in0, s, nullptr,
+                                                 nullptr, 0, &d_n0)))
+            return rc;
+    } else {
+        k_order_keys<<<dim3(grid_for(n)), dim3(256), 0, s>>>(G.vpos, n, key, val);
+        if ((rc = sort_pairs(key, val, key2, val2, n, ctg_bits, sort_tmp, &in0, s, nullptr, nullptr))) return rc;
+        uint32_t *ks = in0 ? key : key2, *ko = in0 ? key2 : key;
+        uint64_t *vs = in0 ? val : val2, *vo = in0 ? val2 : val;
+        unsigned long long *d_cnt = (unsigned long long *)sort_tmp;
+        PAG_HIP_TRY(hipMemsetAsync(d_cnt, 0, 8, s));
+        k_zero_prefix<<<dim3(grid_for(n)), dim3(256), 0, s>>>(ks, n, d_cnt);
+        PAG_HIP_TRY(hipMemcpyAsync(&n0, d_cnt, 8, hipMemcpyDeviceToHost, s));
+        PAG_HIP_TRY(hipStreamSynchronize(s));
+        if (n0 > 1) {
+            k_order_refkeys<<<dim3(grid_for(n0)), dim3(256), 0, s>>>(vs, n0, ks);
+            int in0b = 1;
+            if ((rc = sort_pairs(ks, vs, ko, vo, n0, ref_bits, sort_tmp, &in0b, s, nullptr, nullptr))) return rc;
+            if (!in0b) PAG_HIP_TRY(hipMemcpyAsync(vs, vo, n0 * 8, hipMemcpyDeviceToDevice, s));
+        }
+        k_order_unpack<<<dim3(grid_for(n)), dim3(256), 0, s>>>(ks, vs, n, n0 > 1 ? n0 : 0, G);
+    }
     {
         uint32_t lg = n >= (32ull << 20) ? 3u : 0u;
         if (const long long want = env_int("PAG_ORDER_SLICES", 0)) {
@@ -528,9 +572,14 @@
         if (lg >= bits) lg = 0;
         const uint32_t shift = lg ? bits - lg : 32u;
         for (uint32_t sl = 0; sl < (1u << lg); ++sl)
-            k_order_apply<<<dim3(grid_for(n)), dim3(256), 0, s>>>(ks, vs, n, n0 > 1 ? n0 : 0, G, sl, shift);
+            k_order_apply<<<dim3(grid_for(n)), dim3(256), 0, s>>>(n, G, sl, shift);
     }
     PAG_HIP_TRY(hipGetLastError());
+    if (merged) {
+        PAG_HIP_TRY(hipMemcpyAsync(&n0, d_n0, 8, hipMemcpyDeviceToHost, s));
+        PAG_HIP_TRY(hipStreamSynchronize(s));
+    }
+    if (n_zero) *n_zero = n0;
     return PAG_OK;
 }
 
diff --git a/aligngraph2_amd/csrc/hip/sort_kernels.hpp b/aligngraph2_amd/csrc/hip/sort_kernels.hpp
--- /dev/null
+++ b/aligngraph2_amd/csrc/hip/sort_kernels.hpp
@@ -0,0 +1,412 @@
+#pragma once
+#include <type_traits>
+
+#include "pag_device.hpp"
+
+namespace pagdev {
+
+#ifndef SORT_ST
+#define SORT_ST 1024
+#endif
+#ifndef SORT_ROUNDS
+#define SORT_ROUNDS 5
+#endif
+constexpr int ST = SORT_ST;
+constexpr int SW = ST / 64;
+constexpr int SROUNDS = SORT_ROUNDS;
+constexpr int STILE = ST * SROUNDS;
+constexpr int SMAXR = 256;
+
+struct SortArrayIn {
+    typedef uint32_t A;
+    typedef uint64_t B;
+    typedef uint4 Quad;
+    static __device__ __forceinline__ Quad quad(const A *a, uint64_t base, uint32_t j) { return ((const uint4 *)(a + base))[j]; }
+    static __device__ __forceinline__ void quad_keys(const Quad &x, uint32_t, uint32_t (&k)[4]) {
+        k[0] = x.x;
+        k[1] = x.y;
+        k[2] = x.z;
+        k[3] = x.w;
+    }
+    static __device__ __forceinline__ uint32_t key(const A *a, uint64_t i, uint32_t) { return a[i]; }
+    static __device__ __forceinline__ void rec(const A *a, const B *b, uint64_t i, uint32_t, uint32_t &k, uint64_t &v) {
+        k = a[i];
+        v = b[i];
+    }
+};
+struct SortArrayOut {
+    typedef uint32_t A;
+    typedef uint64_t B;
+    static __device__ __forceinline__ void put(A *a, B *b, uint64_t dst, uint32_t k, uint64_t v, uint32_t) {
+        a[dst] = k;
+        b[dst] = v;
+    }
+};
+
+constexpr int HT = 256;
+constexpr int HW = HT / 64;
+constexpr int HV = STILE / (4 * HT);
+static_assert(STILE % (4 * HT) == 0, "a tile is a whole number of 16-byte loads per thread");
+
+template <class In>
+__global__ __launch_bounds__(HT) void sort_hist(const typename In::A *__restrict__ keys, uint64_t n, int shift, uint32_t rmask,
+                                                uint32_t *__restrict__ hist, uint32_t n_tiles, int aligned, uint32_t pbits) {
+    __shared__ uint32_t h[2][HW][SMAXR];
+    const uint32_t w = threadIdx.x >> 6;
+    typename In::Quad nx[HV];
+    auto request = [&](uint32_t tile) {
+        const uint64_t base = (uint64_t)tile * STILE;
+        if (aligned && tile < n_tiles && base + STILE <= n) {
+#pragma unroll
+            for (int r = 0; r < HV; ++r) nx[r] = In::quad(keys, base, r * HT + threadIdx.x);
+        }
+    };
+    for (uint32_t i = threadIdx.x; i < 2 * HW * SMAXR; i += HT) (&h[0][0][0])[i] = 0;
+    request(blockIdx.x);
+    __syncthreads();
+    uint32_t buf = 0;
+    for (uint32_t tile = blockIdx.x; tile < n_tiles; tile += gridDim.x, buf ^= 1u) {
+        const uint64_t base = (uint64_t)tile * STILE;
+        uint32_t *hw = h[buf][w];
+        if (aligned && base + STILE <= n) {
+            typename In::Quad cur[HV];
+#pragma unroll
+            for (int r = 0; r < HV; ++r) cur[r] = nx[r];
+            request(tile + gridDim.x);
+#pragma unroll
+            for (int r = 0; r < HV; ++r) {
+                uint32_t k[4];
+                In::quad_keys(cur[r], pbits, k);
+                atomicAdd(&hw[(k[0] >> shift) & rmask], 1u);
+                atomicAdd(&hw[(k[1] >> shift) & rmask], 1u);
+                atomicAdd(&hw[(k[2] >> shift) & rmask], 1u);
+                atomicAdd(&hw[(k[3] >> shift) & rmask], 1u);
+            }
+        } else {
+            request(tile + gridDim.x);
+            for (uint32_t j = threadIdx.x; j < (uint32_t)STILE; j += HT)
+                if (base + j < n) atomicAdd(&hw[(In::key(keys, base + j, pbits) >> shift) & rmask], 1u);
+        }
+        __syncthreads();
+        for (uint32_t d = threadIdx.x; d <= rmask; d += HT) {
+            uint32_t c = 0;
+#pragma unroll
+            for (int ww = 0; ww < HW; ++ww) {
+                c += h[buf][ww][d];
+                h[buf][ww][d] = 0;
+            }
+            hist[(uint64_t)d * n_tiles + tile] = c;
+        }
+    }
+}
+
+struct ScatterStage {
+    uint64_t goff[SMAXR];
+    uint32_t skey[STILE];
+#ifdef SORT_TWO_PLANE
+    uint32_t sval_lo[STILE], sval_hi[STILE];
+#else
+    uint64_t sval[STILE];
+#endif
+};
+struct ScatterLds {
+    uint32_t wcnt[SW][SMAXR + 1];
+    uint32_t dstart[SMAXR];
+    ScatterStage stage[2];
+};
+static_assert(SW == 16 || SW == 8, "the wave prefix below scans groups of SW lanes inside a DPP row");
+static_assert(sizeof(ScatterLds) <= 160 * 1024, "LDS");
+static_assert(STILE >= SW * SMAXR, "match words alias the payload staging buffer");
+
+__device__ __forceinline__ uint32_t group_incl_sum(uint32_t v, uint32_t pos) {
+    uint32_t t;
+    t = (uint32_t)__builtin_amdgcn_update_dpp(0, (int)v, 0x111, 0xF, 0xF, true);
+    v += (SW == 16 || pos >= 1u) ? t : 0u;
+    t = (uint32_t)__builtin_amdgcn_update_dpp(0, (int)v, 0x112, 0xF, 0xF, true);
+    v += (SW == 16 || pos >= 2u) ? t : 0u;
+    t = (uint32_t)__builtin_amdgcn_update_dpp(0, (int)v, 0x114, 0xF, 0xF, true);
+    v += (SW == 16 || pos >= 4u) ? t : 0u;
+    if (SW == 16) v += (uint32_t)__builtin_amdgcn_update_dpp(0, (int)v, 0x118, 0xF, 0xF, true);
+    return v;
+}
+
+__device__ __forceinline__ uint64_t scatter_tile(uint32_t block, uint32_t n_blocks, uint32_t it) {
+    if (n_blocks % 8u != 0u) return (uint64_t)it * n_blocks + block;
+    const uint32_t per_xcd = n_blocks / 8u, x = block & 7u, slot = block >> 3;
+    return ((uint64_t)it * 8u + x) * per_xcd + slot;
+}
+
+#ifdef SORT_WAVES_PER_EU
+#define SORT_BOUNDS __launch_bounds__(ST, SORT_WAVES_PER_EU)
+#else
+#define SORT_BOUNDS __launch_bounds__(ST)
+#endif
+template <int BITS, class In = SortArrayIn, class Out = SortArrayOut>
+__global__ SORT_BOUNDS void sort_scatter(const typename In::A *__restrict__ keys, const typename In::B *__restrict__ vals,
+                                         typename Out::A *__restrict__ okeys, typename Out::B *__restrict__ ovals, uint64_t n,
+                                         int shift, const uint64_t *__restrict__ hist_scan, uint32_t n_tiles, uint32_t pbits) {
+    __shared__ ScatterLds L;
+    constexpr uint32_t rmask = (1u << BITS) - 1u;
+    const uint32_t lane = lane_id(), w = threadIdx.x >> 6;
+    const uint32_t n_iter = (n_tiles + gridDim.x - 1) / gridDim.x;
+
+    uint32_t nkey[SROUNDS];
+    uint64_t nval[SROUNDS];
+    uint64_t ngbase = 0;
+    auto request = [&](uint64_t tile) {
+        const uint64_t wb = tile * STILE + (uint64_t)w * (64 * SROUNDS);
+        if (threadIdx.x <= rmask && tile < n_tiles) ngbase = hist_scan[(uint64_t)threadIdx.x * n_tiles + tile];
+#pragma unroll
+        for (int r = 0; r < SROUNDS; ++r) {
+            const uint64_t i = wb + (uint64_t)r * 64 + lane;
+            const bool valid = tile < n_tiles && i < n;
+            nkey[r] = 0u;
+            nval[r] = 0ull;
+            if (valid) In::rec(keys, vals, i, pbits, nkey[r], nval[r]);
+        }
+    };
+    request(scatter_tile(blockIdx.x, gridDim.x, 0));
+
+    const uint32_t last_count = (uint32_t)(n - (uint64_t)(n_tiles - 1u) * STILE);
+    auto staged_val = [&](const ScatterStage &B, uint32_t p) -> uint64_t {
+#ifdef SORT_TWO_PLANE
+        return (uint64_t)B.sval_lo[p] | ((uint64_t)B.sval_hi[p] << 32);
+#else
+        return B.sval[p];
+#endif
+    };
+    auto write_out = [&](const ScatterStage &B, uint32_t count) {
+        if (count == (uint32_t)STILE) {
+#pragma unroll
+            for (int r = 0; r < SROUNDS; ++r) {
+                const uint32_t p = (uint32_t)r * ST + threadIdx.x;
+                const uint32_t kx = B.skey[p];
+                const uint64_t dst = B.goff[(kx >> shift) & rmask] + p;
+                Out::put(okeys, ovals, dst, kx, staged_val(B, p), pbits);
+            }
+        } else {
+            for (uint32_t p = threadIdx.x; p < count; p += ST) {
+                const uint32_t kx = B.skey[p];
+                const uint64_t dst = B.goff[(kx >> shift) & rmask] + p;
+                Out::put(okeys, ovals, dst, kx, staged_val(B, p), pbits);
+            }
+        }
+    };
+
+    bool pending = false;
+    uint32_t pending_count = 0;
+    uint32_t buf = 0;
+    for (uint32_t it = 0; it < n_iter; ++it) {
+        const uint64_t tile = scatter_tile(blockIdx.x, gridDim.x, it);
+        uint32_t key[SROUNDS];
+        uint64_t val[SROUNDS];
+#pragma unroll
+        for (int r = 0; r < SROUNDS; ++r) {
+            key[r] = nkey[r];
+            val[r] = nval[r];
+        }
+        const uint64_t gbase = ngbase;
+        if (it + 1 < n_iter) request(scatter_tile(blockIdx.x, gridDim.x, it + 1));
+        if (pending) write_out(L.stage[buf ^ 1u], pending_count);
+        pending = false;
+        if (tile >= n_tiles) continue;
+
+        ScatterStage &B = L.stage[buf];
+        const uint64_t tile_base = tile * STILE;
+        const uint64_t wave_base = tile_base + (uint64_t)w * (64 * SROUNDS);
+#ifdef SORT_TWO_PLANE
+        unsigned long long *match = (unsigned long long *)&B.sval_lo[0] + (size_t)w * (rmask + 1u);
+#else
+        unsigned long long *match = (unsigned long long *)&B.sval[0] + (size_t)w * (rmask + 1u);
+#endif
+#pragma unroll
+        for (int i = 0; i < SMAXR / 64; ++i) L.wcnt[w][i * 64 + lane] = 0;
+#pragma unroll
+        for (uint32_t i = lane; i <= rmask; i += 64) match[i] = 0ull;
+        uint32_t rk[SROUNDS];
+#pragma unroll
+        for (int r = 0; r < SROUNDS; ++r) {
+            const uint64_t i = wave_base + (uint64_t)r * 64 + lane;
+            const bool valid = i < n;
+            const uint32_t d = (key[r] >> shift) & rmask;
+            if (valid) atomicOr(&match[d], 1ull << lane);
+            const uint64_t peers = valid ? match[d] : 0ull;
+            if (valid) match[d] = 0ull;
+            const uint32_t before = __popcll(peers & lanemask_lt());
+            const uint32_t base = valid ? L.wcnt[w][d] : 0u;
+            if (valid && before == 0) L.wcnt[w][d] = base + (uint32_t)__popcll(peers);
+            rk[r] = base + before;
+        }
+
+        __syncthreads();
+        uint32_t *dtot = (uint32_t *)&B.goff[0];
+#pragma unroll
+        for (int j = 0; j < SMAXR * SW / ST; ++j) {
+            const uint32_t d = (uint32_t)j * (ST / SW) + threadIdx.x / SW, ww = threadIdx.x % SW;
+            const uint32_t c = L.wcnt[ww][d];
+            const uint32_t incl = group_incl_sum(c, ww);
+            L.wcnt[ww][d] = incl - c;
+            if (ww == SW - 1u) dtot[d] = incl;
+        }
+        __syncthreads();
+        if (w == 0) {
+            const uint32_t t0 = dtot[4 * lane], t1 = dtot[4 * lane + 1], t2 = dtot[4 * lane + 2], t3 = dtot[4 * lane + 3];
+            uint32_t tot;
+            const uint32_t ex = wave_excl_sum(t0 + t1 + t2 + t3, &tot);
+            L.dstart[4 * lane] = ex;
+            L.dstart[4 * lane + 1] = ex + t0;
+            L.dstart[4 * lane + 2] = ex + t0 + t1;
+            L.dstart[4 * lane + 3] = ex + t0 + t1 + t2;
+        }
+        __syncthreads();
+#ifdef SORT_LOOKBACK_PROBE
+        if (threadIdx.x <= rmask) {
+            uint32_t *rows = (uint32_t *)(hist_scan + (uint64_t)(rmask + 1u) * n_tiles);
+            __hip_atomic_store(&rows[tile * (rmask + 1u) + threadIdx.x], dtot[threadIdx.x] | 0x40000000u, __ATOMIC_RELAXED, __HIP_MEMORY_SCOPE_AGENT);
+            uint32_t acc = 0;
+            for (uint32_t b = 1; b <= (uint32_t)SORT_LOOKBACK_PROBE; ++b) {
+                const uint64_t t2 = tile >= b ? tile - b : 0;
+                acc += __hip_atomic_load(&rows[t2 * (rmask + 1u) + threadIdx.x], __ATOMIC_RELAXED, __HIP_MEMORY_SCOPE_AGENT);
+            }
+            if (acc == 0xFFFFFFFFu) L.dstart[threadIdx.x] += 1u;
+        }
+        __syncthreads();
+#endif
+        if (threadIdx.x <= rmask) B.goff[threadIdx.x] = gbase - L.dstart[threadIdx.x];
+
+#pragma unroll
+        for (int r = 0; r < SROUNDS; ++r) {
+            const uint64_t i = wave_base + (uint64_t)r * 64 + lane;
+            if (i < n) {
+                const uint32_t d = (key[r] >> shift) & rmask;
+                const uint32_t p = L.dstart[d] + L.wcnt[w][d] + rk[r];
+                B.skey[p] = key[r];
+#ifdef SORT_TWO_PLANE
+                B.sval_lo[p] = (uint32_t)val[r];
+                B.sval_hi[p] = (uint32_t)(val[r] >> 32);
+#else
+                B.sval[p] = val[r];
+#endif
+            }
+        }
+        __syncthreads();
+        pending = true;
+        pending_count = tile == (uint64_t)n_tiles - 1u ? last_count : (uint32_t)STILE;
+        buf ^= 1u;
+    }
+    if (pending) write_out(L.stage[buf ^ 1u], pending_count);
+}
+
+int sort_grids(uint32_t *scatter_blocks, uint32_t *hist_blocks);
+int sort_timing_events(hipEvent_t **ev);
+
+struct SortPass {
+    uint64_t n;
+    uint32_t n_tiles;
+    int shift, bits;
+    uint32_t *hist;
+    uint64_t *hist_scan;
+    void *scan_tmp;
+    uint32_t hist_grid, scatter_grid, pbits;
+    hipStream_t s;
+    hipEvent_t before_scatter, after_scatter;
+};
+template <class In, class Out>
+int sort_pass(const SortPass &p, const typename In::A *ia, const typename In::B *ib, typename Out::A *oa, typename Out::B *ob) {
+    const uint32_t rmask = (1u << p.bits) - 1u;
+    sort_hist<In><<<dim3(p.hist_grid), dim3(HT), 0, p.s>>>(ia, p.n, p.shift, rmask, p.hist, p.n_tiles, ((uintptr_t)ia & 15u) == 0 ? 1 : 0, p.pbits);
+    int rc = scan_u32_to_u64(p.hist, p.hist_scan, (uint64_t)(rmask + 1) * p.n_tiles, nullptr, p.scan_tmp, p.s);
+    if (rc != PAG_OK) return rc;
+    if (p.before_scatter) PAG_HIP_TRY(hipEventRecord(p.before_scatter, p.s));
+    switch (p.bits) {
+#define PAG_SCATTER(B)                                                                                                                              \
+    case B:                                                                                                                                         \
+        sort_scatter<B, In, Out><<<dim3(p.scatter_grid), dim3(ST), 0, p.s>>>(ia, ib, oa, ob, p.n, p.shift, p.hist_scan, p.n_tiles, p.pbits);         \
+        break;
+        PAG_SCATTER(1) PAG_SCATTER(2) PAG_SCATTER(3) PAG_SCATTER(4) PAG_SCATTER(5) PAG_SCATTER(6) PAG_SCATTER(7) PAG_SCATTER(8)
+#undef PAG_SCATTER
+    }
+    if (p.after_scatter) PAG_HIP_TRY(hipEventRecord(p.after_scatter, p.s));
+    return PAG_OK;
+}
+
+template <class In, class Out>
+int sort_passes(const typename In::A *in_a, const typename In::B *in_b, typename Out::A *out_a, typename Out::B *out_b, uint32_t pbits,
+                uint32_t *k0, uint64_t *v0, uint32_t *k1, uint64_t *v1, uint64_t n, int key_bits, void *tmp, int *result_in_0, hipStream_t s,
+                float *ms_dominant_kernel, int *n_passes, int first_bit, const uint64_t **top_clear_dev) {
+    constexpr bool own_in = !std::is_same<In, SortArrayIn>::value, own_out = !std::is_same<Out, SortArrayOut>::value;
+    *result_in_0 = 1;
+    if (ms_dominant_kernel) *ms_dominant_kernel = 0.f;
+    if (n_passes) *n_passes = 0;
+    if (top_clear_dev) *top_clear_dev = nullptr;
+    if (n == 0 || key_bits <= 0) return PAG_OK;
+    uint64_t n_tiles64 = (n + STILE - 1) / STILE;
+    if (n_tiles64 > 0x7FFFFFFFull) {
+        set_error("sort: too many tiles");
+        return PAG_EINVAL;
+    }
+    SortPass p;
+    p.n = n;
+    p.n_tiles = (uint32_t)n_tiles64;
+    p.pbits = pbits;
+    p.s = s;
+    int passes = (key_bits + 7) / 8;
+    int bits = (key_bits + passes - 1) / passes;
+    char *t = (char *)tmp;
+    p.hist = (uint32_t *)t;
+    uint64_t cells = (uint64_t)SMAXR * p.n_tiles;
+    t += (cells * 4 + 255) & ~(size_t)255;
+    p.hist_scan = (uint64_t *)t;
+    t += (cells * 8 + 255) & ~(size_t)255;
+    p.scan_tmp = t;
+
+    uint32_t scatter_blocks = 0, hist_blocks = 0;
+    int rc = sort_grids(&scatter_blocks, &hist_blocks);
+    if (rc != PAG_OK) return rc;
+    p.scatter_grid = p.n_tiles < scatter_blocks ? p.n_tiles : scatter_blocks;
+    p.hist_grid = p.n_tiles < hist_blocks ? p.n_tiles : hist_blocks;
+    const bool timed = ms_dominant_kernel != nullptr;
+    hipEvent_t *ev = nullptr;
+    if (timed && (rc = sort_timing_events(&ev)) != PAG_OK) return rc;
+    uint32_t *ka = own_in ? nullptr : k0, *kb = own_in ? k0 : k1;
+    uint64_t *va = own_in ? nullptr : v0, *vb = own_in ? v0 : v1;
+    int in0 = own_in ? 0 : 1;
+    for (int pass = 0; pass < passes; ++pass) {
+        p.shift = first_bit + pass * bits;
+        p.bits = key_bits - pass * bits < bits ? key_bits - pass * bits : bits;
+        p.before_scatter = timed ? ev[2 * pass] : nullptr;
+        p.after_scatter = timed ? ev[2 * pass + 1] : nullptr;
+        const bool first = own_in && pass == 0, last = own_out && pass == passes - 1;
+        if (first && last)
+            rc = sort_pass<In, Out>(p, in_a, in_b, out_a, out_b);
+        else if (first)
+            rc = sort_pass<In, SortArrayOut>(p, in_a, in_b, kb, vb);
+        else if (last)
+            rc = sort_pass<SortArrayIn, Out>(p, ka, va, out_a, out_b);
+        else
+            rc = sort_pass<SortArrayIn, SortArrayOut>(p, ka, va, kb, vb);
+        if (rc != PAG_OK) return rc;
+        uint32_t *nk = kb == k0 ? k1 : k0;
+        uint64_t *nv = vb == v0 ? v1 : v0;
+        ka = kb, va = vb;
+        kb = nk, vb = nv;
+        in0 = !in0;
+    }
+    PAG_HIP_TRY(hipGetLastError());
+    if (top_clear_dev) *top_clear_dev = p.hist_scan + ((uint64_t)1 << (p.bits - 1)) * p.n_tiles;
+    if (timed) {
+        PAG_HIP_TRY(hipStreamSynchronize(s));
+        float tot = 0.f;
+        for (int pass = 0; pass < passes; ++pass) {
+            float ms = 0.f;
+            PAG_HIP_TRY(hipEventElapsedTime(&ms, ev[2 * pass], ev[2 * pass + 1]));
+            tot += ms;
+        }
+        *ms_dominant_kernel = tot / passes;
+    }
+    if (n_passes) *n_passes = passes;
+    *result_in_0 = in0;
+    return PAG_OK;
+}
+
+}
```
